# fanzhongyi/ExploreMultiModal

Measured on AMD Instinct MI355X. Metric: image-text pairs/sec fwd+bwd, VLMo-Base, 1/2/4/8 MI355X; % bf16 MFMA roofline, higher is better.
Workload: dtype bf16

## Files before the change

### exploremultimodal_amd/csrc/attention.hip

```cpp
#include "common.h"
#include "vlmo_hip.h"

namespace {

struct AttnArgs {
    const bf16* qkv;
    const bf16* ctx;
    const bf16* dctx;
    bf16* out;
    float* lse;
    float* qvsum;
    const int32_t* seg;
    const int32_t* keymask;
    int lse_stride, heads, d;
    float scale, scale_log2e;
    uint32_t drop_thresh, drop_cmp;
    float inv_keep;
    uint64_t seed;
    int bh0;
};

#define LOG2E 1.4426950408889634f
#define LN2 0.6931471805599453f

__device__ __forceinline__ int att_off(int row, int ch) {
    return 1024 * (row >> 3) + 512 * (ch >> 2) + 64 * (row & 7) + 16 * ((ch & 3) ^ ((row >> 2) & 3));
}

template <int NWAVES>
__device__ __forceinline__ void stage_image(const bf16* base, int ld, int col0, const int* rowidx, char* img, int ninstr,
                                            int wave, int lane) {
    const int chhi = lane >> 5, rowlo = (lane >> 2) & 7, pc = lane & 3;
    for (int ii = wave; ii < ninstr; ii += NWAVES) {
        const int row = ii * 8 + rowlo;
        const int ch = chhi * 4 + (pc ^ ((row >> 2) & 3));
        glds16(base + (size_t)rowidx[row] * ld + col0 + ch * 8, img + ii * 1024);
    }
}

#define ATT_G 0x9E3779B1u
#define ATT_G512 ((uint32_t)(512ull * ATT_G))
__device__ __forceinline__ uint32_t att_key(uint64_t seed, int bh) {
    return hash32((uint32_t)seed ^ ((uint32_t)bh * 0x9E3779B9u)) + (uint32_t)(seed >> 32);
}
__device__ __forceinline__ uint32_t att_mix(uint32_t x) {
    x ^= x >> 15;
    x *= 0x7feb352du;
    return x;
}

__device__ __forceinline__ bf16x8 row_frag(const char* img, int row_base, int ks, int lane) {
    return *(const bf16x8*)(img + att_off(row_base + (lane & 31), 2 * ks + (lane >> 5)));
}
__device__ __forceinline__ bf16x8 tr_frag(const char* img, int rb, int cb, int lane) {
    const int g = lane >> 4, q = (lane >> 2) & 3, pp = lane & 3, h = lane >> 5;
    const int col = cb + 16 * (g & 1) + 4 * pp;
    const int r0 = rb + 4 * h + q;
    const bf16x4 lo = lds_tr4<bf16>(img + att_off(r0, col >> 3) + (col & 7) * 2);
    const bf16x4 hi = lds_tr4<bf16>(img + att_off(r0 + 8, col >> 3) + (col & 7) * 2);
    return bf16x8{lo[0], lo[1], lo[2], lo[3], hi[0], hi[1], hi[2], hi[3]};
}

__device__ __forceinline__ f32x16 zero16() {
    f32x16 z;
#pragma unroll
    for (int i = 0; i < 16; ++i) z[i] = 0.f;
    return z;
}

struct SeqRows {
    int rowA, lenA, rowB, N;
    __device__ __forceinline__ SeqRows(const int32_t* seg, int sidx)
        : rowA(seg[4 * sidx + 0]), lenA(seg[4 * sidx + 1]), rowB(seg[4 * sidx + 2]), N(seg[4 * sidx + 1] + seg[4 * sidx + 3]) {}
    __device__ __forceinline__ SeqRows(const int32_t* seg, int sidx, int cap)
        : rowA(seg[4 * sidx + 0]), lenA(min(max(seg[4 * sidx + 1], 0), cap)), rowB(seg[4 * sidx + 2]),
          N(lenA + min(max(seg[4 * sidx + 3], 0), cap - lenA)) {
        if (N == 0) rowA = 1;
    }
    __device__ __forceinline__ int row(int tok) const {
        tok = min(tok, N - 1);
        return tok < lenA ? rowA + tok : rowB + (tok - lenA);
    }
};

__device__ __forceinline__ float key_bias(const int32_t* keymask, int row, int i, int N) {
    return (i < N && (!keymask || keymask[row] != 0)) ? 0.f : -INFINITY;
}

__device__ __forceinline__ void setup_rows(const SeqRows& sr, const int32_t* keymask, int npad, int* rowidx, float* kbias) {
    for (int i = threadIdx.x; i < npad; i += blockDim.x) {
        const int row = sr.row(i);
// ... 377 lines not shown

__device__ __forceinline__ float half_wave_total(float v) {
    float s_ = v + dpp_mov<0x111, 0xf, 0xf>(v);
    s_ += dpp_mov<0x112, 0xf, 0xf>(v);
    s_ += dpp_mov<0x113, 0xf, 0xf>(v);
    s_ += dpp_mov<0x114, 0xf, 0xe>(s_);
    s_ += dpp_mov<0x118, 0xf, 0xc>(s_);
    s_ += dpp_mov<0x142, 0xa, 0xf>(s_);
    return s_;
}
__device__ __forceinline__ void colsum_tile(const f32x16& t, float w, float scale, float* acc, int lane) {
    const int h = lane >> 5;
#pragma unroll
    for (int r = 0; r < 16; ++r) {
        const float v = half_wave_total(t[r] * w);
        if ((lane & 31) == 31) atomicAdd(acc + (r & 3) + 8 * (r >> 2) + 4 * h, v * scale);
    }
}
__device__ __forceinline__ void colsum_tiles(const f32x16* t, float w, float scale, float* acc, int lane) {
#pragma unroll
    for (int dt = 0; dt < 2; ++dt) colsum_tile(t[dt], w, scale, acc + dt * 32, lane);
}

__device__ __forceinline__ int slot_off(int k, int q) {
    return k * 64 + ((((q >> 2) ^ (k >> 1)) & 7) << 3) + (q & 3) * 2;
}
template <bool FRINGE>
__global__ __launch_bounds__(512) void attn_bwd1_kernel(const AttnArgs a, const int NPAD) {
    const int IMG = NPAD * 128;
    extern __shared__ __attribute__((aligned(16))) char smem[];
    char* Qimg = smem;
    char* Dimg = smem + IMG;
    char* Kimg = smem + 2 * IMG;
    const int nt = NPAD >> 5;
    char* slots = smem + 3 * IMG;
    float* kbias = (float*)(slots + 2 * nt * 2048);
    float* nlq = kbias + NPAD;
    float* ndl = nlq + NPAD;
    float* csum = ndl + NPAD;
    char* V8img = (char*)(csum + 128);

    const int lane = threadIdx.x & 63;
    const int w = __builtin_amdgcn_readfirstlane(threadIdx.x >> 6);
    const int nw = blockDim.x >> 6;
    const int bh = blockIdx.x, sidx = bh / a.heads, hd = bh % a.heads;
    const int ld = 3 * a.d;
    const SeqRows sr(a.seg, sidx);
    const int N = sr.N;
    const int nq = (N + 31) >> 5;
    const int nc = FRINGE ? min(nq, 8) : nq;
    for (int ii = w; ii < nq * 4; ii += nw) {
        const int chhi = lane >> 5, rowlo = (lane >> 2) & 7, pc = lane & 3;
        const int row = ii * 8 + rowlo;
        const int ch = chhi * 4 + (pc ^ ((row >> 2) & 3));
        const size_t r = (size_t)sr.row(row);
        glds16(a.qkv + r * ld + hd * 64 + ch * 8, Qimg + ii * 1024);
        glds16(a.qkv + r * ld + a.d + hd * 64 + ch * 8, Kimg + ii * 1024);
        glds16(a.dctx + r * a.d + hd * 64 + ch * 8, Dimg + ii * 1024);
    }
    if (FRINGE && nq > 8 && w >= 4) {
        const int chhi = lane >> 5, rowlo = (lane >> 2) & 7, pc = lane & 3;
        const int row = 256 + (w - 4) * 8 + rowlo;
        const int ch = chhi * 4 + (pc ^ ((row >> 2) & 3));
        glds16(a.qkv + (size_t)sr.row(row) * ld + 2 * a.d + hd * 64 + ch * 8, V8img + (w - 4) * 1024);
    }
    const int l31 = lane & 31, h = lane >> 5;
    const bool active = w < nc;
    const int ki = w * 32 + l31;
    const int krow = sr.row(ki);
    bf16x8 vf[4];
    if (active) {
        const bf16* kp = a.qkv + (size_t)krow * ld + a.d + hd * 64 + 8 * h;
#pragma unroll
        for (int s = 0; s < 4; ++s) vf[s] = *(const bf16x8*)(kp + a.d + 16 * s);
    }
    for (int i = threadIdx.x; i < 128; i += blockDim.x) csum[i] = 0.f;
    const float keep_prob = 1.f / a.inv_keep;
    const float inv_scale = 1.f / a.scale;
    for (int i = threadIdx.x; i < NPAD; i += blockDim.x) {
        float dl = 0.f, lq = INFINITY;
        const int row = sr.row(i);
        const float kb = key_bias(a.keymask, row, i, N);
        if (i < N) {
            const size_t o = (size_t)row * a.d + hd * 64;
            bf16x8 x[8], y[8];
#pragma unroll
            for (int c = 0; c < 8; ++c) {
                x[c] = *(const bf16x8*)(a.ctx + o + 8 * c);
                y[c] = *(const bf16x8*)(a.dctx + o + 8 * c);
            }
            lq = a.lse[(size_t)bh * a.lse_stride + i];
#pragma unroll
            for (int c = 0; c < 8; ++c)
#pragma unroll
                for (int j = 0; j < 8; ++j) dl += (float)x[c][j] * (float)y[c][j];
        }
        kbias[i] = kb;
        ndl[i] = -dl * keep_prob;
        nlq[i] = -lq * inv_scale;
    }
    asm volatile("s_waitcnt vmcnt(0)" ::: "memory");
    __syncthreads();

    const uint32_t akey = att_key(a.seed, bh + a.bh0);
    const float out_scale = a.scale * a.inv_keep;
    const float c_l2 = a.scale_log2e;
    const float kb_own = kbias[min(ki, NPAD - 1)];
    const uint32_t rl_own = (uint32_t)ki * ATT_G + akey + (uint32_t)(4 * h) * ATT_G512;
    f32x16 dK[2] = {zero16(), zero16()}, dV[2] = {zero16(), zero16()}, dQ[2] = {zero16(), zero16()};

    const int xq = (l31 >> 2) & 3;
    const int rf0 = 1024 * (l31 >> 3) + 64 * (l31 & 7) + 16 * (h ^ xq);
    const int rf1 = 1024 * (l31 >> 3) + 64 * (l31 & 7) + 16 * ((2 + h) ^ xq);
    const int tg = (lane >> 4) & 1, tq = (lane >> 2) & 3, tp = lane & 3;
    const int trl = 64 * (4 * h + tq) + 16 * ((2 * tg + (tp >> 1)) ^ h) + 8 * (tp & 1);
    const int trh = 1024 + 64 * (4 * h + tq) + 16 * ((2 * tg + (tp >> 1)) ^ ((2 + h) & 3)) + 8 * (tp & 1);
    auto rfrag = [&](const char* img_rb, int s) __attribute__((always_inline)) -> bf16x8 {
        return *(const bf16x8*)(img_rb + 512 * (s >> 1) + ((s & 1) ? rf1 : rf0));
    };
    auto tfrag = [&](const char* img_rb, int dt) __attribute__((always_inline)) -> bf16x8 {
        const bf16x4 lo = lds_tr4<bf16>(img_rb + 512 * dt + trl);
        const bf16x4 hi = lds_tr4<bf16>(img_rb + 512 * dt + trh);
        return bf16x8{lo[0], lo[1], lo[2], lo[3], hi[0], hi[1], hi[2], hi[3]};
    };
    const int sw0 = slot_off(l31, 4 * h), sw1 = slot_off(l31, 8 + 4 * h);
    const int srl = slot_off(4 * h + tq, 16 * tg + 4 * tp), srh = slot_off(8 + 4 * h + tq, 16 * tg + 4 * tp);
    auto sfrag = [&](const char* slot, int s2) __attribute__((always_inline)) -> bf16x8 {
        const bf16x4 lo = lds_tr4<bf16>(slot + 1024 * s2 + srl);
        const bf16x4 hi = lds_tr4<bf16>(slot + 1024 * s2 + srh);
        return bf16x8{lo[0], lo[1], lo[2], lo[3], hi[0], hi[1], hi[2], hi[3]};
    };

    bf16x8 qa[4], da[4], pf[2], sf[2];
    f32x16 S, dP;
    auto fetch_a = [&](int qt_) __attribute__((always_inline)) {
#pragma unroll
        for (int s = 0; s < 4; ++s) {
            qa[s] = rfrag(Qimg + qt_ * 4096, s);
            da[s] = rfrag(Dimg + qt_ * 4096, s);
        }
    };
    auto qtile = [&](int t_) __attribute__((always_inline)) {
        int q_ = w + t_;
        return q_ >= nc ? q_ - nc : q_;
    };
    auto stage_sdp = [&](int qt, const char* ktile, const bf16x8 (&vfr)[4]) __attribute__((always_inline)) {
        dP = zero16();
#pragma unroll
        for (int g4 = 0; g4 < 4; ++g4) {
            const f32x4 l4 = *(const f32x4*)(nlq + qt * 32 + 8 * g4 + 4 * h);
#pragma unroll
            for (int e = 0; e < 4; ++e) S[4 * g4 + e] = l4[e];
        }
#pragma unroll
        for (int s = 0; s < 4; ++s) {
            S = Elem<bf16>::mfma(qa[s], rfrag(ktile, s), S);
            dP = Elem<bf16>::mfma(da[s], vfr[s], dP);
        }
        __builtin_amdgcn_sched_barrier(0);
    };
    auto stage_valu_dvdk = [&](int qt, char* myslot, float kb, uint32_t rl, f32x16 (&dV)[2],
                               f32x16 (&dK)[2]) __attribute__((always_inline)) {
        bf16x8 dtr[2], qtr[2];
#pragma unroll
        for (int dt = 0; dt < 2; ++dt) {
            dtr[dt] = tfrag(Dimg + qt * 4096, dt);
            qtr[dt] = tfrag(Qimg + qt * 4096, dt);
        }
        __builtin_amdgcn_sched_barrier(0);
        if (a.drop_thresh) {
            const uint32_t rqt = rl + (uint32_t)(qt * 32) * ATT_G512;
#pragma unroll
            for (int g4 = 0; g4 < 4; ++g4) {
                const f32x4 nd = *(const f32x4*)(ndl + qt * 32 + 8 * g4 + 4 * h);
#pragma unroll
                for (int e = 0; e < 4; ++e) {
                    const int i = 4 * g4 + e;
                    const float p = __builtin_amdgcn_exp2f(fmaf(S[i], c_l2, kb));
// ... 175 lines not shown
        }
        __syncthreads();
        if (w < 4) add(w);
        if (w >= 1 && w < 4) put(w);
        __syncthreads();
        if (w == 0) {
            add(1), add(2), add(3);
            if (k8 < N) {
                store_tile(dK, out_scale, row8, a.d);
                store_tile(dV, a.inv_keep, row8, 2 * a.d);
            }
            if (a.qvsum) colsum_tiles(dV, wt8, a.inv_keep, csum + 64, lane);
        }
    } else if (active && ki < N) {
        bf16* op = a.out + (size_t)krow * ld + hd * 64 + 4 * h;
#pragma unroll
        for (int dt = 0; dt < 2; ++dt)
#pragma unroll
            for (int g4 = 0; g4 < 4; ++g4) {
                bf16x4 oq = {(bf16)(dQ[dt][4 * g4 + 0] * out_scale), (bf16)(dQ[dt][4 * g4 + 1] * out_scale),
                             (bf16)(dQ[dt][4 * g4 + 2] * out_scale), (bf16)(dQ[dt][4 * g4 + 3] * out_scale)};
                bf16x4 ok = {(bf16)(dK[dt][4 * g4 + 0] * out_scale), (bf16)(dK[dt][4 * g4 + 1] * out_scale),
                             (bf16)(dK[dt][4 * g4 + 2] * out_scale), (bf16)(dK[dt][4 * g4 + 3] * out_scale)};
                bf16x4 ov = {(bf16)(dV[dt][4 * g4 + 0] * a.inv_keep), (bf16)(dV[dt][4 * g4 + 1] * a.inv_keep),
                             (bf16)(dV[dt][4 * g4 + 2] * a.inv_keep), (bf16)(dV[dt][4 * g4 + 3] * a.inv_keep)};
                *(bf16x4*)(op + dt * 32 + 8 * g4) = oq;
                *(bf16x4*)(op + a.d + dt * 32 + 8 * g4) = ok;
                *(bf16x4*)(op + 2 * a.d + dt * 32 + 8 * g4) = ov;
            }
    }
    if (a.qvsum) {
        if (active && !(FRINGE && nq > 8)) {
            const float wt = ki < N ? 1.f : 0.f;
            colsum_tiles(dQ, wt, out_scale, csum, lane);
            colsum_tiles(dV, wt, a.inv_keep, csum + 64, lane);
        }
        __syncthreads();
        for (int i = threadIdx.x; i < 128; i += blockDim.x) {
            float* dst = a.qvsum + (size_t)sidx * 2 * a.d + (i >> 6) * a.d + hd * 64 + (i & 63);
            *dst = csum[i];
        }
    }
}

#define ATT_LW 8
#define ATT_LCH 4
#define ATT_LBUF (ATT_LCH * 4096)
#define ATT_LMAX 1024
#define ATT_LDS_FWD (4 * ATT_LBUF + ATT_LMAX * 4)
#define ATT_LDS_BWD (4 * ATT_LBUF + 3 * ATT_LMAX * 4 + ATT_LW * 64 * 4)

__device__ __forceinline__ uint32_t att_stride(int N) { return N > 512 ? 1024u : 512u; }

__device__ __forceinline__ void stage_chunk(const bf16* pa, int lda, const bf16* pb, int ldb, const SeqRows& sr, int t0,
                                            int nt, char* ia, char* ib, int w, int lane) {
    const int chhi = lane >> 5, rowlo = (lane >> 2) & 7, pc = lane & 3;
    for (int ii = w; ii < nt * 4; ii += ATT_LW) {
        const int row = t0 * 32 + ii * 8 + rowlo;
        const int ch = chhi * 4 + (pc ^ ((row >> 2) & 3));
        const size_t r = (size_t)sr.row(row);
        glds16(pa + r * lda + ch * 8, ia + ii * 1024);
        glds16(pb + r * ldb + ch * 8, ib + ii * 1024);
    }
}

__device__ __forceinline__ void colsum_wave(const f32x16* t, float wt, float* part, int lane) {
    const int h = lane >> 5;
#pragma unroll
    for (int dt = 0; dt < 2; ++dt)
#pragma unroll
        for (int r = 0; r < 16; ++r) {
            const float v = half_wave_total(t[dt][r] * wt);
            if ((lane & 31) == 31) part[dt * 32 + (r & 3) + 8 * (r >> 2) + 4 * h] += v;
        }
}

__device__ __forceinline__ void bwd_row_constants(const AttnArgs& a, const SeqRows& sr, int bh, int hd, int npad,
                                                  float* lseq, float* delta, float* kbias) {
    const float keep_prob = 1.f / a.inv_keep;
    for (int i = threadIdx.x; i < npad; i += blockDim.x) {
        float dl = 0.f, lq = INFINITY;
        const int row = sr.row(i);
        if (i < sr.N) {
            const size_t o = (size_t)row * a.d + hd * 64;
            bf16x8 x[8], y[8];
#pragma unroll
            for (int c = 0; c < 8; ++c) {
                x[c] = *(const bf16x8*)(a.ctx + o + 8 * c);
                y[c] = *(const bf16x8*)(a.dctx + o + 8 * c);
            }
            lq = a.lse[(size_t)bh * a.lse_stride + i] * LOG2E;
#pragma unroll
            for (int c = 0; c < 8; ++c)
#pragma unroll
                for (int j = 0; j < 8; ++j) dl += (float)x[c][j] * (float)y[c][j];
        }
        delta[i] = dl * keep_prob;
        lseq[i] = lq;
        if (kbias) kbias[i] = key_bias(a.keymask, row, i, sr.N);
    }
}

__global__ __launch_bounds__(512) void attn_fwd_long_kernel(const AttnArgs a) {
    extern __shared__ __attribute__((aligned(16))) char smem[];
    char* ring = smem;
    float* kbias = (float*)(smem + 4 * ATT_LBUF);

    const int lane = threadIdx.x & 63;
    const int w = __builtin_amdgcn_readfirstlane(threadIdx.x >> 6);
    const int bh = blockIdx.x, sidx = bh / a.heads, hd = bh % a.heads;
    const int ld = 3 * a.d;
    const SeqRows sr(a.seg, sidx);
    const int N = sr.N;
    if (N <= 0) return;
    const int nq = (N + 31) >> 5, nch = (nq + ATT_LCH - 1) / ATT_LCH, nrounds = (nq + ATT_LW - 1) / ATT_LW;
    const bf16* kb0 = a.qkv + a.d + hd * 64;
    const bf16* vb0 = a.qkv + 2 * a.d + hd * 64;
    stage_chunk(kb0, ld, vb0, ld, sr, 0, min(ATT_LCH, nq), ring, ring + ATT_LBUF, w, lane);
    for (int i = threadIdx.x; i < nq * 32; i += blockDim.x) kbias[i] = key_bias(a.keymask, sr.row(i), i, N);

    const int l31 = lane & 31, h = lane >> 5;
    const uint32_t akey = att_key(a.seed, bh + a.bh0);
    const uint32_t stride = att_stride(N);
    int qi = 0, qrow = 0;
    uint32_t rq = 0;
    bf16x8 qf[4];
    float m_run = -INFINITY, l_run = 0.f;
    f32x16 O[2] = {zero16(), zero16()};
    const int nsteps = nrounds * nch;
    for (int j = 0; j < nsteps; ++j) {
        const int rd = j / nch, c = j - rd * nch;
        asm volatile("s_waitcnt vmcnt(0)" ::: "memory");
        __syncthreads();
        if (j + 1 < nsteps) {
            const int t0 = ((j + 1) % nch) * ATT_LCH;
            char* nb = ring + ((j + 1) & 1) * 2 * ATT_LBUF;
            stage_chunk(kb0, ld, vb0, ld, sr, t0, min(ATT_LCH, nq - t0), nb, nb + ATT_LBUF, w, lane);
        }
        const char* Kc = ring + (j & 1) * 2 * ATT_LBUF;
        const char* Vc = Kc + ATT_LBUF;
        const int qt = rd * ATT_LW + w;
        if (qt >= nq) continue;
        if (c == 0) {
            qi = qt * 32 + l31;
            qrow = sr.row(qi);
            rq = ((uint32_t)qi * stride + 4u * h) * ATT_G + akey;
            const bf16* qp = a.qkv + (size_t)qrow * ld + hd * 64 + 8 * h;
#pragma unroll
            for (int s = 0; s < 4; ++s) qf[s] = *(const bf16x8*)(qp + 16 * s);
            m_run = -INFINITY, l_run = 0.f;
            O[0] = zero16(), O[1] = zero16();
        }
        const int c0 = c * ATT_LCH;
        f32x16 S[ATT_LCH];
        float mx = -INFINITY;
#pragma unroll
        for (int cc = 0; cc < ATT_LCH; ++cc) {
            S[cc] = zero16();
            const int kt = c0 + cc;
            if (kt < nq) {
#pragma unroll
                for (int s = 0; s < 4; ++s) S[cc] = Elem<bf16>::mfma(row_frag(Kc, cc * 32, s, lane), qf[s], S[cc]);
#pragma unroll
                for (int g4 = 0; g4 < 4; ++g4) {
                    const f32x4 kb = *(const f32x4*)(kbias + kt * 32 + 8 * g4 + 4 * h);
#pragma unroll
                    for (int e = 0; e < 4; ++e) {
                        const float t = S[cc][4 * g4 + e] * a.scale_log2e + kb[e];
                        S[cc][4 * g4 + e] = t;
                        mx = fmaxf(mx, t);
                    }
                }
            }
        }
        mx = fmaxf(mx, __shfl_xor(mx, 32, 64));
        const float m_new = fmaxf(m_run, mx);
        const bool dead = (m_new == -INFINITY);
        const float alpha = dead ? 1.f : __builtin_amdgcn_exp2f(m_run - m_new);
// ... 486 lines not shown
}

int check_common(const char* fn, const void* qkv, const int32_t* seg, int num_seq, int heads, int d, int max_len,
                 int cap) {
    VLMO_CHECK_ARG(qkv && seg, "%s: null pointer", fn);
    VLMO_CHECK_ARG(num_seq > 0 && heads > 0, "%s: empty problem", fn);
    VLMO_CHECK_ARG(d == heads * 64, "%s: head_dim must be 64 (d=%d, heads=%d)", fn, d, heads);
    VLMO_CHECK_ARG(max_len > 0 && max_len <= cap, "%s: sequence length %d exceeds this build's limit %d", fn, max_len, cap);
    return 0;
}

AttnArgs make_args(const void* qkv, const int32_t* seg, const int32_t* keymask, const float* lse, int lse_stride, int heads,
                   int d, float scale, uint32_t drop_thresh, float inv_keep, uint64_t seed, int mask_seq0) {
    AttnArgs a{};
    a.qkv = (const bf16*)qkv;
    a.lse = (float*)lse;
    a.seg = seg;
    a.keymask = keymask;
    a.lse_stride = lse_stride;
    a.heads = heads;
    a.d = d;
    a.scale = scale;
    a.scale_log2e = scale * LOG2E;
    a.drop_thresh = drop_thresh;
    a.drop_cmp = drop_thresh >= 65536u ? 0xFFFFFFFFu : drop_thresh << 16;
    a.inv_keep = drop_thresh ? inv_keep : 1.f;
    a.seed = seed;
    a.bh0 = mask_seq0 * heads;
    return a;
}

int run_map(const char* fn, const void* qkv, const void* dctx, const int32_t* seg, int num_seq, const int32_t* keymask,
            float* out, int heads, int d, int seq_len, int q0, int nq, int kind, int head_mean, float scale,
            hipStream_t stream) {
    if (int rc = check_common(fn, qkv, seg, num_seq, heads, d, seq_len, ATT_LMAX)) return rc;
    VLMO_CHECK_ARG(q0 >= 0 && nq >= 1 && q0 <= seq_len - nq, "%s: query rows [%d, %d + %d) outside [0, %d)", fn, q0, q0, nq,
                   seq_len);
    MapArgs a{};
    a.qkv = (const bf16*)qkv;
    a.dctx = (const bf16*)dctx;
    a.seg = seg;
    a.keymask = keymask;
    a.out = out;
    a.heads = heads;
    a.d = d;
    a.seq_len = seq_len;
    a.q0 = q0;
    a.nq = nq;
    a.kind = kind;
    a.head_mean = head_mean != 0;
    a.scale_log2e = scale * LOG2E;
    const int gx = num_seq * (a.head_mean ? 1 : heads);
    const int rounds = ((nq + 31) / 32 + ATT_PW - 1) / ATT_PW;
    const int gy = std::min(rounds, std::max(1, (768 + gx - 1) / gx));
    a.tiles_per_block = ATT_PW * ((rounds + gy - 1) / gy);
    launch_map(a, gx, (rounds * ATT_PW + a.tiles_per_block - 1) / a.tiles_per_block, stream);
    VLMO_CHECK_LAUNCH(fn);
    return 0;
}

}

extern "C" int vlmo_attn_fwd(const void* qkv, const int32_t* seg, int num_seq, const int32_t* keymask, void* ctx,
                             float* lse, int lse_stride, int heads, int d, int max_len, float scale,
                             uint32_t drop_thresh, float inv_keep, uint64_t seed, int mask_seq0, hipStream_t stream) {
    if (int rc = check_common("vlmo_attn_fwd", qkv, seg, num_seq, heads, d, max_len, 1024)) return rc;
    VLMO_CHECK_ARG(ctx, "vlmo_attn_fwd: null ctx");
    VLMO_CHECK_ARG(!lse || lse_stride >= max_len, "vlmo_attn_fwd: lse_stride too small");
    AttnArgs a = make_args(qkv, seg, keymask, lse, lse_stride, heads, d, scale, drop_thresh, inv_keep, seed, mask_seq0);
    a.out = (bf16*)ctx;
    const int nt = (max_len + 31) / 32, nb = num_seq * heads;
    if (max_len > 512) {
        launch_fwd_long(a, nb, stream);
        VLMO_CHECK_LAUNCH("vlmo_attn_fwd(long)");
        return 0;
    }
    if (nt == 9) launch_fwd1_fringe(a, max_len, nb, stream);
    else if (nt < 9) launch_fwd1(a, nt, nb, stream);
    else launch_fwd(a, nt, nb, stream);
    VLMO_CHECK_LAUNCH("vlmo_attn_fwd");
    return 0;
}

extern "C" int vlmo_attn_bwd(const void* qkv, const void* ctx, const void* dctx, const float* lse, int lse_stride,
                             const int32_t* seg, int num_seq, const int32_t* keymask, void* dqkv, float* qv_colsum,
                             int heads, int d, int max_len, float scale, uint32_t drop_thresh, float inv_keep,
                             uint64_t seed, int mask_seq0, hipStream_t stream) {
    if (int rc = check_common("vlmo_attn_bwd", qkv, seg, num_seq, heads, d, max_len, 1024)) return rc;
    VLMO_CHECK_ARG(ctx && dctx && lse && dqkv, "vlmo_attn_bwd: null pointer");
    VLMO_CHECK_ARG(lse_stride >= max_len, "vlmo_attn_bwd: lse_stride too small");
    AttnArgs a = make_args(qkv, seg, keymask, lse, lse_stride, heads, d, scale, drop_thresh, inv_keep, seed, mask_seq0);
    a.ctx = (const bf16*)ctx;
    a.dctx = (const bf16*)dctx;
    a.out = (bf16*)dqkv;
    a.qvsum = qv_colsum;
    const int nt = (max_len + 31) / 32, nb = num_seq * heads;
    if (max_len > 288) {
        launch_bwd_long(a, nb, stream);
        VLMO_CHECK_LAUNCH("vlmo_attn_bwd(long)");
        return 0;
    }
    const int rc = nt > 8 ? launch_bwd1<true>(a, nt, nb, stream) : launch_bwd1<false>(a, nt, nb, stream);
    VLMO_CHECK_ARG(rc == 0, "vlmo_attn_bwd: %d tokens do not fit the LDS of one CU", max_len);
    VLMO_CHECK_LAUNCH("vlmo_attn_bwd");
    return 0;
}

extern "C" int vlmo_attn_probs(const void* qkv, const int32_t* seg, int num_seq, const int32_t* keymask, float* probs,
                               int heads, int d, int seq_len, int q0, int nq, int head_mean, float scale,
                               hipStream_t stream) {
    VLMO_CHECK_ARG(probs, "vlmo_attn_probs: null probs");
    return run_map("vlmo_attn_probs", qkv, nullptr, seg, num_seq, keymask, probs, heads, d, seq_len, q0, nq, 0, head_mean,
                   scale, stream);
}

extern "C" int vlmo_attn_gradcam(const void* qkv, const void* dctx, const int32_t* seg, int num_seq, const int32_t* keymask,
                                 float* out, int heads, int d, int seq_len, int q0, int nq, int kind, int head_mean,
                                 float scale, hipStream_t stream) {
    VLMO_CHECK_ARG(dctx && out, "vlmo_attn_gradcam: null dctx or out");
    VLMO_CHECK_ARG(kind == VLMO_GRADCAM_CAM || kind == VLMO_GRADCAM_ATTN_GRAD || kind == VLMO_GRADCAM_GRAD,
                   "vlmo_attn_gradcam: unknown kind %d", kind);
    return run_map("vlmo_attn_gradcam", qkv, dctx, seg, num_seq, keymask, out, heads, d, seq_len, q0, nq, kind, head_mean,
                   scale, stream);
}
```

### exploremultimodal_amd/csrc/block.hip

```cpp
#include "common.h"
#include "vlmo_hip.h"
#include <algorithm>
#include <map>
#include <vector>

namespace {
constexpr int GELU_DERIV = 4;


struct Events {
    std::vector<hipEvent_t> pool;
    hipEvent_t get(size_t i) {
        while (pool.size() <= i) {
            hipEvent_t e = nullptr;
            (void)hipEventCreateWithFlags(&e, hipEventDisableTiming);
            pool.push_back(e);
        }
        return pool[i];
    }
};
Events& events() {
    static thread_local std::map<int, Events> per_device;
    int dev = 0;
    (void)hipGetDevice(&dev);
// ... 69 lines not shown
        w2[x] = b->w2[x];
        VlmoEpilogue& f = e2[x] = epi();
        f.out = bp(b->x2, r0, d, 4);
        f.ldo = d;
        f.out2 = b->need_bwd ? bp(b->zd2, r0, d, 2) : nullptr;
        f.ld2 = d;
        f.bias = b->b2[x];
        f.gamma = b->g2;
        f.resid = (const float*)bp((const void*)b->x1, r0, d, 4);
        f.row_scale = b->row_index ? b->rs2 : (b->rs2 ? b->rs2 + r0 : nullptr);
        f.row_index = b->row_index ? b->row_index + r0 : nullptr;
        f.drop_thresh = b->drop_thresh;
        f.inv_keep = b->inv_keep;
        f.seed = b->seed + 21 + 2 * x;
    }
    TRY(vlmo_gemm_nt_grouped(VLMO_EPI_BIAS_GELU, VLMO_BF16, b->tile, b->n_experts, a1, d, w1, d, rows, hid, d, e1, st));
    TRY(vlmo_gemm_nt_grouped(VLMO_EPI_RESID, VLMO_BF16, b->tile, b->n_experts, a2, hid, w2, hid, rows, d, hid, e2, st));
    return 0;
}

}

extern "C" int vlmo_side_stream_create(int low_priority, const uint32_t* cu_mask, int cu_mask_words, hipStream_t* out) {
    VLMO_CHECK_ARG(out, "vlmo_side_stream_create: null out");
    hipError_t rc;
    if (cu_mask && cu_mask_words > 0) {
        rc = hipExtStreamCreateWithCUMask(out, (uint32_t)cu_mask_words, cu_mask);
    } else {
        int least = 0, greatest = 0;
        (void)hipDeviceGetStreamPriorityRange(&least, &greatest);
        rc = hipStreamCreateWithPriority(out, hipStreamNonBlocking, low_priority ? least : 0);
    }
    if (rc != hipSuccess) {
        vlmo_set_error("vlmo_side_stream_create: %s", hipGetErrorString(rc));
        return (int)rc;
    }
    return 0;
}

namespace {

struct Deferred {
    std::vector<VlmoTnProblem> tn;
    std::vector<VlmoColJob> col;
    std::vector<int> blocks;
    bool store = false;
};

void push_col(Deferred& D, const VlmoColJob& j) {
    if (j.src && j.rows > 0) D.col.push_back(j);
}
void push_tn(Deferred& D, const void* A, int lda, const void* B, int ldb, float* C, int ldc, int M, int N1, int N2) {
    D.tn.push_back(VlmoTnProblem{A, B, C, lda, ldb, ldc, M, N1, N2, 1.f, D.store ? 0 : 1});
}

struct StackWs {
    int64_t ln2;
    int64_t resid[2];
    int64_t ln1;
    int64_t colpart;
    int64_t qv;
    int64_t total;
    int64_t slot;
};
StackWs stack_ws_layout(int M, int d, int hidden, int max_seqs) {
    StackWs w{};
    w.slot = reduce_ws_need(2 * d) / 4;
    w.ln2 = 0;
    w.resid[0] = w.ln2 + 2 * w.slot;
    w.resid[1] = w.resid[0] + w.slot;
    w.ln1 = w.resid[1] + w.slot;
    w.colpart = w.ln1 + 2 * w.slot;
    w.qv = w.colpart + (int64_t)((M + 15) / 16 + 1) * hidden;
    w.total = w.qv + (int64_t)max_seqs * 2 * d;
    return w;
}
int block_seqs(const VlmoBlockDesc* b) {
    int n = 0;
    for (int a = 0; a < b->n_attn; ++a) n += b->nseq[a];
    return n;
}

int check_block_bwd(const VlmoBlockDesc* b, int i) {
    VLMO_CHECK_ARG(b->dx2 && b->dx1 && b->dx0, "vlmo_stack_bwd: block %d: null gradient buffers", i);
    VLMO_CHECK_ARG(b->n_experts >= 1 && b->n_experts <= 2 && b->n_attn >= 1 && b->n_attn <= 2,
                   "vlmo_stack_bwd: block %d: 1..2 experts and attention launches per block", i);
    VLMO_CHECK_ARG(b->M > 0 && b->exp_rows[0] >= 0 && (b->n_experts == 1 || b->exp_rows[1] >= 0) &&
                       (int64_t)b->exp_rows[0] + (b->n_experts == 2 ? b->exp_rows[1] : 0) <= b->M,
                   "vlmo_stack_bwd: block %d: expert rows exceed M = %d", i, b->M);
    const int64_t need = stack_ws_layout(b->M, b->d, b->hidden, block_seqs(b)).total * 4;
    VLMO_CHECK_ARG(b->ws_main && b->ws_bytes >= need,
                   "vlmo_stack_bwd: block %d: column workspace of %lld bytes is too small: need %lld bytes = "
                   "vlmo_stack_bwd_ws_bytes(%d, %d, %d, %d)",
                   i, (long long)b->ws_bytes, (long long)need, b->M, b->d, b->hidden, block_seqs(b));
    return 0;
}

int block_dgrad_chain(const VlmoBlockDesc* b, hipStream_t st, Deferred& D, const VlmoBlockDesc* below, bool skip_resid,
                      bool* fused_below) {
    const int M = b->M, d = b->d, hid = b->hidden;
    const int nseq_all = block_seqs(b);
    const StackWs W = stack_ws_layout(M, d, hid, nseq_all);
    const int64_t slot_bytes = W.slot * 4;
    float* const ws = b->ws_main;
    const void *ag[4], *wg[4], *af[4], *wf[4];
    int32_t rows[4];
    VlmoEpilogue eg[4], ef[4];
    float* colpart = ws + W.colpart;
    for (int x = 0; x < b->n_experts; ++x) {
        const size_t r0 = b->exp_row0[x];
        const int n = rows[x] = b->exp_rows[x];
        if (!skip_resid) {
            VlmoColJob fold{};
            TRY(resid_bwd_launch(b->dx2 + r0 * d, bp(b->zd2, r0, d, 2), b->g2,
                                 b->row_index ? b->rs2 : (b->rs2 ? b->rs2 + r0 : nullptr),
                                 b->row_index ? b->row_index + r0 : nullptr, bp(b->dz2, r0, d, 2), b->dg2, b->db2[x], n, d,
                                 b->drop_thresh, b->inv_keep, b->seed + 21 + 2 * x, ws + W.resid[x], slot_bytes, &fold, st));
            push_col(D, fold);
        }
        ag[x] = bp(b->dz2, r0, d, 2);
        wg[x] = b->w2T[x];
        VlmoEpilogue& e = eg[x] = epi();
        e.out = bp(b->du, r0, hid, 2);
        e.ldo = hid;
        e.aux = bp(b->u, r0, hid, 2);
        e.ld2 = hid;
        e.drop_thresh = b->drop_thresh;
        e.inv_keep = b->inv_keep;
        e.seed = b->seed + 20 + 2 * x;
        e.relu = GELU_DERIV;
        if (b->db1[x]) {
            const int nblk16 = (n + 15) / 16;
            e.colpart = colpart;
            push_col(D, fold_job(colpart, hid, nblk16, hid, hid, b->db1[x]));
            colpart += (int64_t)nblk16 * hid;
        }
        af[x] = bp(b->du, r0, hid, 2);
        wf[x] = b->w1T[x];
        VlmoEpilogue& f = ef[x] = epi();
        f.out = bp(b->dy2, r0, d, 2);
        f.ldo = d;
        push_tn(D, bp(b->dz2, r0, d, 2), d, bp(b->h, r0, hid, 2), hid, b->dw2[x], hid, n, d, hid);
        push_tn(D, bp(b->du, r0, hid, 2), hid, bp(b->y2, r0, d, 2), d, b->dw1[x], d, n, hid, d);
    }
    TRY(vlmo_gemm_nt_grouped(VLMO_EPI_DGELU, VLMO_BF16, b->tile, b->n_experts, ag, d, wg, d, rows, hid, d, eg, st));
    TRY(vlmo_gemm_nt_grouped(VLMO_EPI_BIAS, VLMO_BF16, b->tile, b->n_experts, af, hid, wf, hid, rows, d, hid, ef, st));
    {
        VlmoColJob fold{};
        TRY(ln_bwd_fold(b->dy2, b->x1, b->n2w, b->mean2, b->rstd2, b->dx2, b->dx1, b->dn2w, b->dn2b, b->zd1, b->g1, b->rs1,
                        b->row_index, b->dz1, b->dg1, b->dproj_b, b->drop_thresh, b->inv_keep, b->seed + 1, M, d, ws + W.ln2,
                        2 * slot_bytes, &fold, st));
        push_col(D, fold);
    }
    {
        VlmoEpilogue e = epi();
        e.out = b->dctx;
        e.ldo = d;
        TRY(vlmo_gemm_nt(VLMO_EPI_BIAS, VLMO_BF16, b->tile, b->dz1, d, b->proj_wT, d, M, d, d, &e, st));
    }
    const float scale = 1.0f / sqrtf((float)(d / b->heads));
    float* const qvsum = ws + W.qv;
    for (int a = 0, s0 = 0; a < b->n_attn; s0 += b->nseq[a], ++a)
        TRY(vlmo_attn_bwd(b->qkv, b->ctx, b->dctx, b->lse[a], b->lse_stride[a], b->seg[a], b->nseq[a], b->keymask,
                          b->dqkv, qvsum + (size_t)s0 * 2 * d, b->heads, d, b->maxlen[a], scale, b->attn_drop_thresh,
                          b->attn_inv_keep, b->seed + 11 + b->attn_seed_idx[a], b->attn_seq0[a], st));
    push_tn(D, b->dz1, d, b->ctx, d, b->dproj_w, d, M, d, d);
    push_tn(D, b->dqkv, 3 * d, b->y1, d, b->dqkv_w, d, M, 3 * d, d);
    push_col(D, fold_job(qvsum, 2 * d, nseq_all, 2 * d, d, b->dqkv_b, b->dqkv_b + 2 * d));
    {
        VlmoEpilogue e = epi();
        e.out = b->dy1;
        e.ldo = d;
        TRY(vlmo_gemm_nt(VLMO_EPI_BIAS, VLMO_BF16, b->tile, b->dqkv, 3 * d, b->qkv_wT, 3 * d, M, d, 3 * d, &e, st));
    }
    const VlmoBlockDesc* n = below;
    *fused_below = n && n->M == M && n->d == d && n->dx2 == b->dx0 && n->zd2 && n->dz2 && n->exp_row0[0] == 0 &&
                   (n->n_experts == 1 ? n->exp_rows[0] == M
                                      : (n->exp_row0[1] == n->exp_rows[0] && n->exp_rows[0] + n->exp_rows[1] == M));
    VlmoColJob fold{};
    if (*fused_below) {
        const int seg = n->n_experts == 1 ? M : n->exp_row0[1];
        float* wsf = ws + W.ln1;
        int nb0 = 0;
        TRY(ln_resid_seg_bwd(b->dy1, b->x, b->n1w, b->mean1, b->rstd1, b->dx1, b->dx0, b->dn1w, b->dn1b, n->zd2, n->g2,
                             n->rs2, n->row_index, n->dz2, n->dg2, n->drop_thresh, n->inv_keep, n->seed + 21, n->seed + 23,
                             seg, M, d, wsf, 2 * slot_bytes, &fold, &nb0, st));
        push_col(D, fold);
        if (n->db2[0]) push_col(D, fold_job(wsf + 3 * d, 4 * d, nb0, d, d, n->db2[0]));
        if (n->n_experts == 2 && n->db2[1])
            push_col(D, fold_job(wsf + 3 * d + (size_t)nb0 * 4 * d, 4 * d, fold.rows - nb0, d, d, n->db2[1]));
    } else {
        TRY(ln_bwd_fold(b->dy1, b->x, b->n1w, b->mean1, b->rstd1, b->dx1, b->dx0, b->dn1w, b->dn1b, nullptr, nullptr, nullptr,
                        nullptr, nullptr, nullptr, nullptr, 0, 1.f, 0, M, d, ws + W.ln1, slot_bytes, &fold, st));
        push_col(D, fold);
    }
    return 0;
}

}

extern "C" int64_t vlmo_stack_bwd_ws_bytes(int M, int d, int hidden, int max_seqs) {
    return stack_ws_layout(M, d, hidden, max_seqs).total * 4;
}

extern "C" int vlmo_stack_fwd(const VlmoStackDesc* s, hipStream_t st) {
    VLMO_CHECK_ARG(s && s->blocks && s->n_blocks >= 1, "vlmo_stack_fwd: empty stack");
    for (int i = 0; i < s->n_blocks; ++i)
        if (int rc = block_fwd(&s->blocks[i], st)) return rc;
    return 0;
}

extern "C" int vlmo_stack_bwd(const VlmoStackDesc* s, hipStream_t st) {
    VLMO_CHECK_ARG(s && s->blocks && s->n_blocks >= 1, "vlmo_stack_bwd: empty stack");
    const int nb = s->n_blocks;
    for (int i = 0; i < nb; ++i) TRY(check_block_bwd(&s->blocks[i], i));
    const int batch = s->wgrad_batch >= 1 ? s->wgrad_batch : 1;
    const int nsets = s->n_tmp_sets >= 1 ? s->n_tmp_sets : 1;
    hipStream_t side = s->side_stream ? s->side_stream : st;
    const bool two = side != st;
    VLMO_CHECK_ARG(!two || nsets > batch || nb <= nsets,
                   "vlmo_stack_bwd: %d temporary sets cannot cover deferred batches of %d blocks", nsets, batch);
    Events& ev = events();
    Deferred D;
    D.store = s->wgrad_store != 0;
    std::vector<int> batch_of(nb, -1);
    int n_batches = 0, waited_upto = -1;
    auto flush = [&]() -> int {
        if (D.blocks.empty()) return 0;
        if (two) {
            hipEvent_t f = ev.get(2 * n_batches);
            (void)hipEventRecord(f, st);
            (void)hipStreamWaitEvent(side, f, 0);
        }
        std::stable_sort(D.tn.begin(), D.tn.end(), [](const VlmoTnProblem& a, const VlmoTnProblem& b) { return a.M > b.M; });
        TRY(vlmo_gemm_tn_multi(VLMO_BF16, D.tn.data(), (int)D.tn.size(), side));
        TRY(vlmo_colwork_multi(VLMO_BF16, D.col.data(), (int)D.col.size(), side));
        if (two) (void)hipEventRecord(ev.get(2 * n_batches + 1), side);
        if (s->grad_ready)
            for (int i : D.blocks)
                if (s->grad_ready[i]) (void)hipEventRecord((hipEvent_t)s->grad_ready[i], side);
        ++n_batches;
        D.tn.clear();
        D.col.clear();
        D.blocks.clear();
        return 0;
    };
    auto set_free = [&](int kk) -> int {
        if (!two || kk < nsets || kk >= nb) return 0;
// ... 44 lines not shown
```

### exploremultimodal_amd/csrc/common.h

```cpp
#pragma once
#include <hip/hip_runtime.h>
#include <stdint.h>
#include <type_traits>
#include "vlmo_hip.h"

typedef __bf16 bf16;
typedef _Float16 f16;
typedef __attribute__((ext_vector_type(8))) __bf16 bf16x8;
typedef __attribute__((ext_vector_type(4))) __bf16 bf16x4;
typedef __attribute__((ext_vector_type(2))) __bf16 bf16x2;
typedef __attribute__((ext_vector_type(8))) _Float16 f16x8;
typedef __attribute__((ext_vector_type(4))) _Float16 f16x4;
typedef __attribute__((ext_vector_type(16))) float f32x16;
typedef __attribute__((ext_vector_type(4))) float f32x4;
typedef __attribute__((ext_vector_type(2))) float f32x2;

#define LDS_PTR(p) ((__attribute__((address_space(3))) void*)(p))
#define GLB_PTR(p) ((const __attribute__((address_space(1))) void*)(p))

void vlmo_set_error(const char* fmt, ...);
#define VLMO_CHECK_ARG(cond, ...)                         \
    do {                                                  \
        if (!(cond)) {                                    \
            vlmo_set_error(__VA_ARGS__);                  \
// ... 84 lines not shown
#endif
    __device__ __forceinline__ void init(const void* base) {
#if defined(__HIP_DEVICE_COMPILE__)
        r = __builtin_amdgcn_make_buffer_rsrc((void*)base, 0, 0x7FFFFFFF, 0x00020000);
#endif
    }
    __device__ __forceinline__ void load16(void* lds_wave_base, uint32_t lane_off, int scalar_off) const {
#if defined(__HIP_DEVICE_COMPILE__)
        __builtin_amdgcn_raw_ptr_buffer_load_lds(r, LDS_PTR(lds_wave_base), 16, lane_off, scalar_off, 0, 0);
#endif
    }
};

template <typename T>
__device__ __forceinline__ typename Elem<T>::v4 lds_tr4(const void* p);
template <>
__device__ __forceinline__ bf16x4 lds_tr4<bf16>(const void* p) {
    return __builtin_amdgcn_ds_read_tr16_b64_v4bf16(
        (__attribute__((address_space(3))) bf16x4*)(p));
}
template <>
__device__ __forceinline__ f16x4 lds_tr4<f16>(const void* p) {
    typedef __attribute__((__vector_size__(4 * sizeof(__fp16)))) __fp16 hv4;
    const hv4 r = __builtin_amdgcn_ds_read_tr16_b64_v4f16((__attribute__((address_space(3))) hv4*)(p));
    return __builtin_bit_cast(f16x4, r);
}

__device__ __forceinline__ uint32_t hash32(uint32_t x) {
    x ^= x >> 16;
    x *= 0x7feb352du;
    x ^= x >> 15;
    x *= 0x846ca68bu;
    x ^= x >> 16;
    return x;
}
__device__ __forceinline__ uint32_t drop_half(uint64_t seed, uint64_t group_idx, int half) {
    const uint32_t i = (uint32_t)(group_idx * 2 + half);
    return hash32((i ^ (uint32_t)seed) * 0x9E3779B9u + (uint32_t)(seed >> 32));
}
__device__ __forceinline__ uint64_t drop_bits4(uint64_t seed, uint64_t group_idx) {
    return (uint64_t)drop_half(seed, group_idx, 0) | ((uint64_t)drop_half(seed, group_idx, 1) << 32);
}
__device__ __forceinline__ bool drop_keep(uint64_t bits, int j, uint32_t thresh) {
    return ((uint32_t)(bits >> (16 * j)) & 0xFFFFu) >= thresh;
}
__device__ __forceinline__ bool drop_keep1(uint64_t seed, uint64_t group_idx, int j, uint32_t thresh) {
    return ((drop_half(seed, group_idx, j >> 1) >> (16 * (j & 1))) & 0xFFFFu) >= thresh;
}

__device__ __forceinline__ float norm_cdf_from(float x, float e) {
    const float t = __builtin_amdgcn_rcpf(fmaf(0.3275911f * 0.70710678118654752f, fabsf(x), 1.0f));
    float poly = fmaf(0.5f * 1.061405429f, t, 0.5f * -1.453152027f);
    poly = fmaf(poly, t, 0.5f * 1.421413741f);
    poly = fmaf(poly, t, 0.5f * -0.284496736f);
    poly = fmaf(poly, t, 0.5f * 0.254829592f);
    const float tail = poly * t * e;
    return x >= 0.f ? 1.0f - tail : tail;
}
__device__ __forceinline__ float gauss_from(float x) {
    return __builtin_amdgcn_exp2f(x * x * -0.72134752044448170f);
}
__device__ __forceinline__ float gelu_erf(float x) {
    const float e = gauss_from(x);
    return x * norm_cdf_from(x, e);
}
__device__ __forceinline__ float gelu_erf_grad(float x) {
    const float e = gauss_from(x);
    return norm_cdf_from(x, e) + x * 0.39894228040143268f * e;
}

template <int CTRL, int ROW_MASK, int BANK_MASK> __device__ __forceinline__ float dpp_mov(float v) {
    return __builtin_bit_cast(float, __builtin_amdgcn_update_dpp(0, __builtin_bit_cast(int, v), CTRL, ROW_MASK, BANK_MASK, false));
}
__device__ __forceinline__ float wave_sum(float v) {
    float s = v + dpp_mov<0x111, 0xf, 0xf>(v);
    s += dpp_mov<0x112, 0xf, 0xf>(v);
    s += dpp_mov<0x113, 0xf, 0xf>(v);
    s += dpp_mov<0x114, 0xf, 0xe>(s);
    s += dpp_mov<0x118, 0xf, 0xc>(s);
    s += dpp_mov<0x142, 0xa, 0xf>(s);
    s += dpp_mov<0x143, 0xc, 0xf>(s);
    return __builtin_bit_cast(float, __builtin_amdgcn_readlane(__builtin_bit_cast(int, s), 63));
}
__device__ __forceinline__ float wave_max(float v) {
#pragma unroll
    for (int o = 32; o > 0; o >>= 1) v = fmaxf(v, __shfl_xor(v, o, 64));
    return v;
}
```

### exploremultimodal_amd/csrc/gemm_common.h

```cpp
#pragma once
#include "common.h"
#include "vlmo_hip.h"

namespace {

struct GemmNT {
    const void* A;
    const void* B;
    int M, N, K, lda, ldb;
    VlmoEpilogue e;
    int cH, cW, cCin, ckw;
    const void* zero;
    int group_m;
    const void* A2;
    int lda2, k1;
    float seg_scale;
};

constexpr int MAX_GROUPS = 4;
struct GemmNTGroups {
    int ngroups;
    int t0[MAX_GROUPS + 1];
    GemmNT g[MAX_GROUPS];
};

struct RowAddr {
    size_t base;
    uint32_t off;
    template <typename U> __device__ __forceinline__ U* at(const void* p) const {
        return (U*)((char*)((U*)p + base) + off * (uint32_t)sizeof(U));
    }
};
template <typename T, bool NT = true> __device__ __forceinline__ void store4(T* p, float a, float b, float c, float d) {
    typedef typename Elem<T>::v4 v4;
    const v4 v = {(T)a, (T)b, (T)c, (T)d};
    if constexpr (NT)
        __builtin_nontemporal_store(v, (v4*)p);
    else
        *(v4*)p = v;
}
#define NT_LD(p) __builtin_nontemporal_load(p)
template <typename T> __device__ __forceinline__ f32x4 load4(const T* p);
template <> __device__ __forceinline__ f32x4 load4<bf16>(const bf16* p) {
    bf16x4 v = NT_LD((const bf16x4*)p);
    return f32x4{(float)v[0], (float)v[1], (float)v[2], (float)v[3]};
}
template <> __device__ __forceinline__ f32x4 load4<f16>(const f16* p) {
    f16x4 v = NT_LD((const f16x4*)p);
    return f32x4{(float)v[0], (float)v[1], (float)v[2], (float)v[3]};
}

__device__ __forceinline__ void pin4(f32x4& v) {
    asm volatile("" : "+v"(v[0]), "+v"(v[1]), "+v"(v[2]), "+v"(v[3]));
}

template <typename T, int EPI, int GD = -1>
__device__ __forceinline__ f32x4 epilogue4(const GemmNT& p, int gmb, int row, int gn, f32x4 v, f32x4 bias4,
                                           f32x4 gamma4, f32x4 ext, float rs, bool ok) {
    const VlmoEpilogue& e = p.e;
    v += bias4;
    const int gm = gmb + row;
    const RowAddr o{(size_t)gmb * e.ldo, (uint32_t)(row * e.ldo + gn)};
    const RowAddr o2{(size_t)gmb * e.ld2, (uint32_t)(row * e.ld2 + gn)};
    if constexpr (EPI == VLMO_EPI_BIAS) {
        const float lo = (e.relu & 1) ? 0.f : -INFINITY;
#pragma unroll
        for (int j = 0; j < 4; ++j) v[j] = fmaxf(v[j], lo);
        pin4(v);
        if (ok) store4<T>(o.at<T>(e.out), v[0], v[1], v[2], v[3]);
    } else if constexpr (EPI == VLMO_EPI_F32) {
        if (e.beta != 0.f) v += e.beta * ext;
        pin4(v);
        if (ok) *(f32x4*)o.at<float>(e.out) = v;
    } else if constexpr (EPI == VLMO_EPI_BIAS_GELU) {
        f32x4 h;
        if (GD >= 0 ? GD != 0 : (e.relu & 4) != 0) {
#pragma unroll
            for (int j = 0; j < 4; ++j) {
                const float u = v[j], ee = gauss_from(u), cdf = norm_cdf_from(u, ee);
                h[j] = u * cdf;
                v[j] = fmaf(u * 0.39894228040143268f, ee, cdf);
            }
            if (e.drop_thresh) {
                const uint64_t bits = drop_bits4(e.seed, ((uint64_t)gm * p.N + gn) >> 2);
#pragma unroll
                for (int j = 0; j < 4; ++j) {
                    const float m = drop_keep(bits, j, e.drop_thresh) ? e.inv_keep : 0.f;
                    h[j] *= m;
                    v[j] *= m;
                }
            }
        } else {
#pragma unroll
            for (int j = 0; j < 4; ++j) h[j] = gelu_erf(v[j]);
            if (e.drop_thresh) {
                const uint64_t bits = drop_bits4(e.seed, ((uint64_t)gm * p.N + gn) >> 2);
#pragma unroll
                for (int j = 0; j < 4; ++j) h[j] = drop_keep(bits, j, e.drop_thresh) ? h[j] * e.inv_keep : 0.f;
            }
        }
        pin4(v);
        pin4(h);
        if (ok) {
            store4<T>(o.at<T>(e.out), v[0], v[1], v[2], v[3]);
            store4<T>(o2.at<T>(e.out2), h[0], h[1], h[2], h[3]);
        }
    } else if constexpr (EPI == VLMO_EPI_RESID) {
        if (e.drop_thresh) {
            const uint64_t bits = drop_bits4(e.seed, ((uint64_t)gm * p.N + gn) >> 2);
#pragma unroll
            for (int j = 0; j < 4; ++j) v[j] = drop_keep(bits, j, e.drop_thresh) ? v[j] * e.inv_keep : 0.f;
        }
        f32x4 x2 = ext + gamma4 * v * rs;
        pin4(v);
        pin4(x2);
        if (ok) {
            if (e.out2) store4<T>(o2.at<T>(e.out2), v[0], v[1], v[2], v[3]);
            *(f32x4*)o.at<float>(e.out) = x2;
        }
    } else if constexpr (EPI == VLMO_EPI_DUAL) {
        v = v * e.beta + ext;
        pin4(v);
        if (ok) {
            store4<T>(o.at<T>(e.out), v[0], v[1], v[2], v[3]);
            if (e.out2)
                store4<T>((T*)e.out2 + (size_t)gm * e.ld2 + gn, fmaxf(v[0], 0.f), fmaxf(v[1], 0.f), fmaxf(v[2], 0.f),
                          fmaxf(v[3], 0.f));
        }
    } else if constexpr (EPI == VLMO_EPI_CE_BWD) {
        const int gmc = min(gm, p.M - 1);
        const float lse = e.resid[gmc], sc = e.row_scale[gmc];
        const int lab = e.row_index[gmc];
#pragma unroll
        for (int j = 0; j < 4; ++j)
            v[j] = (__builtin_amdgcn_exp2f((v[j] - lse) * 1.4426950408889634f) - (gn + j == lab ? 1.f : 0.f)) * sc;
        pin4(v);
        if (ok) store4<T>(o.at<T>(e.out), v[0], v[1], v[2], v[3]);
    } else if constexpr (EPI == VLMO_EPI_DGELU) {
        if (GD >= 0 ? GD != 0 : (e.relu & 4) != 0) {
            v *= ext;
        } else {
#pragma unroll
            for (int j = 0; j < 4; ++j) v[j] *= gelu_erf_grad(ext[j]);
            if (e.drop_thresh) {
                const uint64_t bits = drop_bits4(e.seed, ((uint64_t)gm * p.N + gn) >> 2);
#pragma unroll
                for (int j = 0; j < 4; ++j) v[j] = drop_keep(bits, j, e.drop_thresh) ? v[j] * e.inv_keep : 0.f;
            }
        }
        pin4(v);
        if (ok) store4<T>(o.at<T>(e.out), v[0], v[1], v[2], v[3]);
    }
    return v;
}

template <typename T, int EPI>
__device__ __forceinline__ f32x4 epilogue_ext(const GemmNT& p, int gmb, int rowc, int gnc) {
    const VlmoEpilogue& e = p.e;
    const f32x4 z = {0.f, 0.f, 0.f, 0.f};
    const RowAddr o{(size_t)gmb * e.ldo, (uint32_t)(rowc * e.ldo + gnc)};
    const RowAddr o2{(size_t)gmb * e.ld2, (uint32_t)(rowc * e.ld2 + gnc)};
    if constexpr (EPI == VLMO_EPI_RESID) {
        return NT_LD((const f32x4*)o.at<float>(e.resid));
    } else if constexpr (EPI == VLMO_EPI_DGELU) {
        return load4<T>(o2.at<T>(e.aux));
    } else if constexpr (EPI == VLMO_EPI_DUAL) {
        return e.resid ? load4<T>(o.at<T>(e.resid)) : z;
    } else if constexpr (EPI == VLMO_EPI_F32) {
        return e.beta != 0.f ? *(const f32x4*)o.at<float>(e.out) : z;
    } else {
        return z;
    }
}

__device__ __forceinline__ const void* uniform_ptr(const void* p) {
    const uint64_t v = (uint64_t)p;
    const uint32_t lo = __builtin_amdgcn_readfirstlane((uint32_t)v), hi = __builtin_amdgcn_readfirstlane((uint32_t)(v >> 32));
    return (const void*)(const __attribute__((address_space(1))) void*)(((uint64_t)hi << 32) | lo);
}

__device__ __forceinline__ int uniform_i(int v) { return __builtin_amdgcn_readfirstlane(v); }
__device__ __forceinline__ float uniform_f(float v) {
    return __builtin_bit_cast(float, __builtin_amdgcn_readfirstlane(__builtin_bit_cast(int, v)));
}

__device__ __forceinline__ int xcd_remap(int bid, int nwg) {
    const int q = nwg >> 3, r = nwg & 7, x = bid & 7;
    const int base = (x < r) ? x * (q + 1) : r * (q + 1) + (x - r) * q;
    return base + (bid >> 3);
}

template <int BK> __device__ __forceinline__ int nt_swz(int row) {
    return BK == 64 ? ((row >> 1) & 7) : ((row >> 2) & 3);
}

template <typename T, int BM, int BN, int WM, int WN, int EPI, bool CONV, int BK, int NSTG, bool PP = false>
__global__ __launch_bounds__(WM * WN * 64, 2) void gemm_nt_kernel(const GemmNTGroups gp) {
    typedef typename Elem<T>::v8 v8;
    constexpr bool SEG2 = __is_same(T, f16) && !CONV;
    constexpr int NW = WM * WN;
    constexpr int TM = BM / WM / 32, TN = BN / WN / 32;
    constexpr int ROWB = BK * 2, CPR = ROWB / 16, SRPI = 1024 / ROWB, KS = BK / 16;
    constexpr int A_BYTES = BM * ROWB, B_BYTES = BN * ROWB, STAGE = A_BYTES + B_BYTES;
    constexpr int NA = BM / SRPI / NW, NB = BN / SRPI / NW;
    static_assert(BM % (SRPI * NW) == 0 && BN % (SRPI * NW) == 0, "tile/wave mismatch");
    static_assert(NW * 32 * TN * 32 * 4 <= NSTG * STAGE, "epilogue LDS must fit in the ring");
    extern __shared__ __attribute__((aligned(16))) char smem[];

    const int tid = threadIdx.x, lane = tid & 63;
    const int wave = __builtin_amdgcn_readfirstlane(tid >> 6);
    const int wm = wave / WN, wn = wave % WN;
    const int lid_all = xcd_remap(blockIdx.x, gridDim.x);
    auto locate = [&](int la, int& gi_, int& m0_, int& n0_) {
        int g = 0;
#pragma unroll
        for (int q = 1; q < MAX_GROUPS; ++q)
            if (q < gp.ngroups && la >= gp.t0[q]) g = q;
        g = __builtin_amdgcn_readfirstlane(g);
        const GemmNT& r = gp.g[g];
        const int M_ = uniform_i(r.M), N_ = uniform_i(r.N);
        const int tiles_n = (N_ + BN - 1) / BN, tiles_m = (M_ + BM - 1) / BM;
        const int lid = la - uniform_i(gp.t0[g]);
        const int gmr = uniform_i(r.group_m);
        const int gm_ = gmr > 0 ? gmr : 1;
        const int per_group = gm_ * tiles_n;
        const int first_m = (lid / per_group) * gm_;
        const int gsz = min(tiles_m - first_m, gm_);
        const int in_g = lid % per_group;
        gi_ = g;
        m0_ = (first_m + in_g % gsz) * BM;
        n0_ = (in_g / gsz) * BN;
    };
    const T* a_src[NA];
    const T* b_src[NB];
    int a_yx[NA];
    auto point = [&](int gi_, int m0_, int n0_) {
        const GemmNT& r = gp.g[gi_];
        const T* A_ = (const T*)uniform_ptr(r.A);
        const T* B_ = (const T*)uniform_ptr(r.B);
        const int M_ = uniform_i(r.M), N_ = uniform_i(r.N), lda_ = uniform_i(r.lda), ldb_ = uniform_i(r.ldb);
#pragma unroll
        for (int i = 0; i < NA; ++i) {
            const int rr = (i * NW + wave) * SRPI + lane / CPR;
            const int c = (lane % CPR) ^ nt_swz<BK>(rr);
            const int gr = min(m0_ + rr, M_ - 1);
            a_src[i] = A_ + (size_t)gr * lda_ + c * 8;
            if constexpr (CONV) {
                const int cH = uniform_i(r.cH), cW = uniform_i(r.cW);
                const int pix = gr % (cH * cW);
                a_yx[i] = ((pix / cW) << 16) | (pix % cW);
            }
        }
#pragma unroll
        for (int i = 0; i < NB; ++i) {
            const int rr = (i * NW + wave) * SRPI + lane / CPR;
// ... 126 lines not shown
            }
        }
    }
    stage(0, 0);
#pragma unroll
    for (int i = 0; i < TM; ++i)
#pragma unroll
        for (int j = 0; j < TN; ++j)
#pragma unroll
            for (int k = 0; k < 16; ++k) acc[i][j][k] = 0.f;
    if constexpr (PP) {
        static_assert(NSTG == 2 && WM == 2 && KS == 4, "ping-pong schedule: 2 buffers, 2 row groups, BK = 64");
        v8 af[2][TM], bf[2][TN];
        auto read_half = [&](const char* s_, int hf) {
#pragma unroll
            for (int q = 0; q < 2; ++q) {
                const int coff = ((2 * (2 * hf + q) + h) ^ swz) << 4;
#pragma unroll
                for (int i = 0; i < TM; ++i) af[q][i] = *(const v8*)(s_ + a_row_off + i * 32 * ROWB + coff);
#pragma unroll
                for (int j = 0; j < TN; ++j) bf[q][j] = *(const v8*)(s_ + b_row_off + j * 32 * ROWB + coff);
            }
            if constexpr (CONV && sizeof(T) == 2 && __is_same(T, f16)) {
                if (pp->e.relu & 2) {
                    const v8 z = {0, 0, 0, 0, 0, 0, 0, 0};
#pragma unroll
                    for (int q = 0; q < 2; ++q)
#pragma unroll
                        for (int i = 0; i < TM; ++i) af[q][i] = __builtin_elementwise_max(af[q][i], z);
                }
            }
        };
        auto mfma_half = [&]() {
            __builtin_amdgcn_s_setprio(1);
#pragma unroll
            for (int q = 0; q < 2; ++q)
#pragma unroll
                for (int i = 0; i < TM; ++i)
#pragma unroll
                    for (int j = 0; j < TN; ++j) acc[i][j] = Elem<T>::mfma(af[q][i], bf[q][j], acc[i][j]);
            __builtin_amdgcn_s_setprio(0);
        };
        auto bar = [&]() {
            __builtin_amdgcn_sched_barrier(0);
            asm volatile("s_waitcnt lgkmcnt(0)" ::: "memory");
            __builtin_amdgcn_s_barrier();
            asm volatile("" ::: "memory");
            __builtin_amdgcn_sched_barrier(0);
        };
        asm volatile("s_waitcnt vmcnt(0)" ::: "memory");
        __builtin_amdgcn_s_barrier();
        if (wm == 1) bar();
        for (int kt = 0; kt < nk; ++kt) {
            const char* cur = smem + (kt & 1) * STAGE;
            const bool more = kt + 1 < nk;
            seg_boundary(kt);
            read_half(cur, 0);
            if (more) stage((kt + 1) & 1, kt + 1);
            bar();
            mfma_half();
            bar();
            read_half(cur, 1);
            if (more && wm == 1) asm volatile("s_waitcnt vmcnt(0)" ::: "memory");
            bar();
            mfma_half();
            if (more && wm == 0) asm volatile("s_waitcnt vmcnt(0)" ::: "memory");
            bar();
        }
        if (wm == 0) bar();
    } else {
        static_assert(NSTG == 2, "two LDS buffers");
        for (int kt = 0; kt < nk; ++kt) {
            asm volatile("s_waitcnt vmcnt(0)" ::: "memory");
            __syncthreads();
            if (kt + 1 < nk) stage((kt + 1) & 1, kt + 1);
            seg_boundary(kt);
            compute(smem + (kt & 1) * STAGE);
        }
    }

    __syncthreads();
    constexpr int ROWF = TN * 32;
    constexpr int LPR = TN * 8, RPI = 64 / LPR;
    float* ep = (float*)(smem + wave * (32 * ROWF * 4));
    const int rrow = lane / LPR, rcol = (lane % LPR) * 4;
    const int gn = n0 + wn * (BN / WN) + rcol;
    const bool col_ok = gn < p.N;
    const int gnc = col_ok ? gn : 0;
    f32x4 bias4 = {0.f, 0.f, 0.f, 0.f}, gamma4 = {1.f, 1.f, 1.f, 1.f};
    if (p.e.bias) bias4 = *(const f32x4*)(p.e.bias + gnc);
    if (EPI == VLMO_EPI_RESID && p.e.gamma) gamma4 = *(const f32x4*)(p.e.gamma + gnc);
    f32x4 csum = {0.f, 0.f, 0.f, 0.f};
#pragma unroll
    for (int i = 0; i < TM; ++i) {
        constexpr int NIT = 32 / RPI;
        const int gmb = __builtin_amdgcn_readfirstlane(m0 + wm * (BM / WM) + i * 32);
        const int gmbc = min(gmb, p.M - 1);
        f32x4 ext[NIT];
        float rs[NIT];
        int ridx[NIT];
#pragma unroll
        for (int it = 0; it < NIT; ++it) {
            const int gmc = gmbc + min(it * RPI + rrow, p.M - 1 - gmbc);
            ridx[it] = (EPI == VLMO_EPI_RESID && p.e.row_scale && p.e.row_index) ? p.e.row_index[gmc] : gmc;
        }
#pragma unroll
        for (int it = 0; it < NIT; ++it) {
            const int rowc = min(it * RPI + rrow, p.M - 1 - gmbc);
            if constexpr (PRE) {
                const typename Elem<T>::v4 q = pre[i][it];
                ext[it] = p.e.resid ? f32x4{(float)q[0], (float)q[1], (float)q[2], (float)q[3]} : f32x4{0.f, 0.f, 0.f, 0.f};
            } else {
                ext[it] = epilogue_ext<T, EPI>(p, gmbc, rowc, gnc);
            }
            rs[it] = (EPI == VLMO_EPI_RESID && p.e.row_scale) ? p.e.row_scale[ridx[it]] : 1.f;
        }
#pragma unroll
        for (int j = 0; j < TN; ++j)
#pragma unroll
            for (int r = 0; r < 16; ++r)
                ep[((r & 3) + 8 * (r >> 2) + 4 * h) * ROWF + j * 32 + l31] = acc[i][j][r];
        __builtin_amdgcn_fence(__ATOMIC_RELEASE, "wavefront");
        __builtin_amdgcn_wave_barrier();
        __builtin_amdgcn_fence(__ATOMIC_ACQUIRE, "wavefront");
        f32x4 v[NIT];
#pragma unroll
        for (int it = 0; it < NIT; ++it) v[it] = *(const f32x4*)(ep + (it * RPI + rrow) * ROWF + rcol);
#pragma unroll
        for (int it = 0; it < NIT; ++it) {
            const int row = it * RPI + rrow;
            const int gm = gmb + row;
            if constexpr (EPI == VLMO_EPI_ARGMAX) {
                f32x4 vv = v[it] + bias4;
                float best = -INFINITY;
                int bi = 0x7fffffff;
#pragma unroll
                for (int j = 0; j < 4; ++j)
                    if (gn + j < p.N && vv[j] > best) {
                        best = vv[j];
                        bi = gn + j;
                    }
#pragma unroll
                for (int o = 1; o < LPR; o <<= 1) {
                    const float ob = __shfl_xor(best, o, 64);
                    const int oi = __shfl_xor(bi, o, 64);
                    if (ob > best || (ob == best && oi < bi)) {
                        best = ob;
                        bi = oi;
                    }
                }
                if ((lane % LPR) == 0 && gm < p.M && col_ok) {
                    const int chunk = (n0 + wn * (BN / WN)) / ROWF;
                    float* pv = (float*)p.e.out + ((size_t)gm * p.e.ldo + chunk) * 2;
                    pv[0] = best;
                    ((int*)pv)[1] = bi;
                }
            } else if constexpr (EPI == VLMO_EPI_CE) {
                f32x4 vv = v[it] + bias4;
                const int lab = (gm < p.M) ? p.e.row_index[gm] : -1;
                float best = -INFINITY, labv = -INFINITY;
                int bi = 0x7fffffff;
#pragma unroll
                for (int j = 0; j < 4; ++j)
                    if (gn + j < p.N) {
                        if (vv[j] > best) {
                            best = vv[j];
                            bi = gn + j;
                        }
                        if (gn + j == lab) labv = vv[j];
                    }
#pragma unroll
                for (int o = 1; o < LPR; o <<= 1) {
                    const float ob = __shfl_xor(best, o, 64);
                    const int oi = __shfl_xor(bi, o, 64);
                    if (ob > best || (ob == best && oi < bi)) {
                        best = ob;
                        bi = oi;
                    }
                    labv = fmaxf(labv, __shfl_xor(labv, o, 64));
                }
                float se = 0.f;
#pragma unroll
                for (int j = 0; j < 4; ++j)
                    if (gn + j < p.N) se += __builtin_amdgcn_exp2f((vv[j] - best) * 1.4426950408889634f);
#pragma unroll
                for (int o = 1; o < LPR; o <<= 1) se += __shfl_xor(se, o, 64);
                if ((lane % LPR) == 0 && gm < p.M && col_ok) {
                    const int chunk = (n0 + wn * (BN / WN)) / ROWF;
                    float* pv = (float*)p.e.out + ((size_t)gm * p.e.ldo + chunk) * 4;
                    pv[0] = best;
                    pv[1] = se;
                    ((int*)pv)[2] = bi;
                    pv[3] = labv;
                }
            } else {
                const bool ok = gm < p.M && col_ok;
                const f32x4 w = epilogue4<T, EPI>(p, gmb, row, gn, v[it], bias4, gamma4, ext[it], rs[it], ok);
                if constexpr (EPI == VLMO_EPI_DGELU) {
#pragma unroll
                    for (int j = 0; j < 4; ++j) csum[j] += ok ? w[j] : 0.f;
                }
            }
        }
        __builtin_amdgcn_fence(__ATOMIC_RELEASE, "wavefront");
        __builtin_amdgcn_wave_barrier();
        __builtin_amdgcn_fence(__ATOMIC_ACQUIRE, "wavefront");
        if constexpr (EPI == VLMO_EPI_DGELU) {
            if (p.e.colpart) {
#pragma unroll
                for (int o = LPR; o < 64; o <<= 1)
#pragma unroll
                    for (int j = 0; j < 4; ++j) csum[j] += __shfl_xor(csum[j], o, 64);
                const int blk = gmb >> 4;
                if (lane < LPR && col_ok && gmb < p.M) {
                    *(f32x4*)(p.e.colpart + (size_t)blk * p.N + gn) = csum;
                    if (gmb + 16 < p.M) *(f32x4*)(p.e.colpart + (size_t)(blk + 1) * p.N + gn) = f32x4{0.f, 0.f, 0.f, 0.f};
                }
                csum = f32x4{0.f, 0.f, 0.f, 0.f};
            }
        }
    }
}

template <typename T, int BM, int BN, int WM, int WN, bool CONV = false, int BK = 64, int NSTG = 2, bool PP = false,
          unsigned EMASK = 0xFFFFFFFFu>
int launch_nt(int epi, GemmNTGroups& p, hipStream_t st) {
    int tiles = 0;
    for (int q = 0; q < p.ngroups; ++q) {
        p.t0[q] = tiles;
        tiles += ((p.g[q].M + BM - 1) / BM) * ((p.g[q].N + BN - 1) / BN);
    }
    for (int q = p.ngroups; q <= MAX_GROUPS; ++q) p.t0[q] = tiles;
    constexpr int LDS = NSTG * (BM + BN) * BK * 2;
    dim3 grid(tiles), block(WM * WN * 64);
#define VLMO_LAUNCH_EPI(E)                                                                     \
    case E:                                                                                    \
    if constexpr (((EMASK >> E) & 1u) == 0) {                                                  \
        known = false;                                                                         \
    } else {                                                                                   \
        auto k = gemm_nt_kernel<T, BM, BN, WM, WN, E, CONV, BK, NSTG, PP>;                                        \
        if (LDS > 65536) {                                                                     \
            static DeviceOnce attr_set;              \
            if (attr_set.first())                                                              \
                (void)hipFuncSetAttribute((const void*)k, hipFuncAttributeMaxDynamicSharedMemorySize, LDS); \
        }                                                                                      \
        hipLaunchKernelGGL(k, grid, block, LDS, st, p);                                        \
    } break;
    bool known = true;
    switch (epi) {
        VLMO_LAUNCH_EPI(VLMO_EPI_BIAS)
        VLMO_LAUNCH_EPI(VLMO_EPI_F32)
        VLMO_LAUNCH_EPI(VLMO_EPI_DUAL)
        default:
            if constexpr (!CONV) {
                switch (epi) {
                    VLMO_LAUNCH_EPI(VLMO_EPI_BIAS_GELU)
                    VLMO_LAUNCH_EPI(VLMO_EPI_RESID)
                    VLMO_LAUNCH_EPI(VLMO_EPI_DGELU)
                    VLMO_LAUNCH_EPI(VLMO_EPI_ARGMAX)
                    VLMO_LAUNCH_EPI(VLMO_EPI_CE)
                    VLMO_LAUNCH_EPI(VLMO_EPI_CE_BWD)
                    default:
                        known = false;
                }
            } else {
                known = false;
            }
    }
    if (!known) {
        vlmo_set_error("vlmo_gemm_nt/conv: unsupported epilogue %d", epi);
        return -1;
    }
#undef VLMO_LAUNCH_EPI
    VLMO_CHECK_LAUNCH("vlmo_gemm_nt");
    return 0;
}

}

namespace vlmo_prof {
struct ProfRec;
struct ProfScope {
    ProfRec* r = nullptr;
    hipStream_t st;
    ProfScope(int tag, double flops, hipStream_t s);
    ~ProfScope();
};
}
using vlmo_prof::ProfScope;

extern "C" __attribute__((visibility("hidden"))) int launch_nt16_height(int h16, int epi, GemmNTGroups& gp,
                                                                        hipStream_t stream);
```

### exploremultimodal_amd/csrc/gemm_nt.hip

```cpp
#include "gemm_common.h"
#include <mutex>
#include <vector>

namespace vlmo_prof {
struct ProfRec {
    hipEvent_t a, b;
    int tag;
    double flops;
};
struct Prof {
    std::vector<ProfRec> recs;
    size_t used = 0;
    bool on = false;
    std::mutex mu;
} g_prof;

ProfScope::ProfScope(int tag, double flops, hipStream_t s) : st(s) {
    if (!g_prof.on) return;
    std::lock_guard<std::mutex> lk(g_prof.mu);
    if (g_prof.used < g_prof.recs.size()) {
        r = &g_prof.recs[g_prof.used++];
        r->tag = tag;
        r->flops = flops;
        (void)hipEventRecord(r->a, st);
    }
}
ProfScope::~ProfScope() {
    if (r) (void)hipEventRecord(r->b, st);
}

extern "C" int vlmo_profile_start(int max_records) {
    std::lock_guard<std::mutex> lk(g_prof.mu);
    while ((int)g_prof.recs.size() < max_records) {
        ProfRec r{};
        if (hipEventCreate(&r.a) != hipSuccess || hipEventCreate(&r.b) != hipSuccess) {
            vlmo_set_error("vlmo_profile_start: hipEventCreate failed");
            return -1;
        }
        g_prof.recs.push_back(r);
    }
    g_prof.used = 0;
    g_prof.on = true;
    return 0;
}

extern "C" int vlmo_profile_stop(int ntags, double* ms, double* flops, int64_t* launches) {
    std::lock_guard<std::mutex> lk(g_prof.mu);
    g_prof.on = false;
    for (int i = 0; i < ntags; ++i) {
        ms[i] = 0;
        flops[i] = 0;
        launches[i] = 0;
    }
    for (size_t i = 0; i < g_prof.used; ++i) {
        const ProfRec& r = g_prof.recs[i];
        float t = 0.f;
        if (r.tag < 0 || r.tag >= ntags || hipEventElapsedTime(&t, r.a, r.b) != hipSuccess) continue;
        ms[r.tag] += t;
        flops[r.tag] += r.flops;
        launches[r.tag] += 1;
    }
    return (int)g_prof.used;
}
}

namespace {
int check_nt(int epi, const void* A, int lda, const void* B, int ldb, int M, int N, int K, const VlmoEpilogue* e) {
    VLMO_CHECK_ARG(A && B && e, "vlmo_gemm_nt: null operand");
    VLMO_CHECK_ARG(M > 0 && N > 0 && K > 0, "vlmo_gemm_nt: empty problem M=%d N=%d K=%d", M, N, K);
    VLMO_CHECK_ARG(K % 64 == 0, "vlmo_gemm_nt: K=%d must be a multiple of 64", K);
    VLMO_CHECK_ARG(N % 4 == 0, "vlmo_gemm_nt: N=%d must be a multiple of 4", N);
    VLMO_CHECK_ARG(lda % 8 == 0 && ldb % 8 == 0 && lda >= K && ldb >= K, "vlmo_gemm_nt: bad lda/ldb %d/%d", lda, ldb);
    VLMO_CHECK_ARG(e->out && (epi == VLMO_EPI_ARGMAX || epi == VLMO_EPI_CE || (e->ldo >= N && e->ldo % 4 == 0)), "vlmo_gemm_nt: bad output / ldo");
    VLMO_CHECK_ARG(epi != VLMO_EPI_CE || (e->ldo >= (N + 63) / 64 && e->row_index), "vlmo_gemm_nt: cross-entropy epilogue needs labels and ldo >= chunks");
    VLMO_CHECK_ARG(epi != VLMO_EPI_CE_BWD || (e->resid && e->row_scale && e->row_index), "vlmo_gemm_nt: cross-entropy backward needs lse, row scale, labels");
    VLMO_CHECK_ARG(epi != VLMO_EPI_BIAS_GELU || (e->out2 && e->ld2 >= N), "vlmo_gemm_nt: gelu epilogue needs out2");
    VLMO_CHECK_ARG(epi != VLMO_EPI_ARGMAX || e->ldo >= (N + 63) / 64, "vlmo_gemm_nt: argmax partial buffer too narrow");
    VLMO_CHECK_ARG(epi != VLMO_EPI_RESID || e->resid, "vlmo_gemm_nt: residual epilogue needs resid");
    VLMO_CHECK_ARG(epi != VLMO_EPI_DGELU || (e->aux && e->ld2 >= N), "vlmo_gemm_nt: dgelu epilogue needs aux");
    return 0;
}

int run_nt(int epi, int dtype, int tile, GemmNTGroups& gp, hipStream_t stream) {
    VLMO_CHECK_ARG(dtype == VLMO_BF16 || dtype == VLMO_F16, "vlmo_gemm_nt: dtype must be bf16 or f16");
    const int tile_in = tile;
    long Mtot = 0;
    for (int q = 0; q < gp.ngroups; ++q) Mtot += gp.g[q].M;
    const int N = gp.g[0].N, K = gp.g[0].K;
    if (tile < 0) {
        tile = (K >= 1536 && Mtot >= 2048 && N >= 512) ? 3 : 0;
        if (tile == 0 && K >= 512 && N >= 512 && Mtot >= 2048) {
            long t256 = 0;
            for (int q = 0; q < gp.ngroups; ++q) t256 += (long)((gp.g[q].M + 255) / 256) * ((N + 255) / 256);
            if (t256 <= 256) tile = 3;
        }
        long t256_all = 0;
        for (int q = 0; q < gp.ngroups; ++q) t256_all += (long)((gp.g[q].M + 255) / 256) * ((N + 255) / 256);
        const bool few_tiles = t256_all <= 128;
        if (few_tiles) tile = 0;
        if (tile == 0 && dtype == VLMO_BF16 && (epi == VLMO_EPI_BIAS || epi == VLMO_EPI_BIAS_GELU) && K <= 1024 && N >= 2048 && Mtot >= 4096)
            tile = 4;
        if (!few_tiles && dtype == VLMO_BF16 && (epi == VLMO_EPI_BIAS || epi == VLMO_EPI_BIAS_GELU || epi == VLMO_EPI_RESID || epi == VLMO_EPI_DGELU) && K >= 1024) {
            long t256 = 0, t192n = 0;
            for (int q = 0; q < gp.ngroups; ++q) {
                t256 += (long)((gp.g[q].M + 255) / 256) * ((N + 255) / 256);
                t192n += (long)((gp.g[q].M + 191) / 192) * ((N + 255) / 256);
            }
            const long e256 = ((t256 + 255) / 256) * 256, e192 = ((t192n + 255) / 256) * 192;
            if (e192 * 10 <= e256 * 9) tile = 8;
        }
    }
    if ((tile == 0 || tile == 3 || tile == 4 || tile == 8) && dtype == VLMO_BF16 && !gp.g[0].k1 && !gp.g[0].ckw &&
        (epi == VLMO_EPI_BIAS || epi == VLMO_EPI_BIAS_GELU || epi == VLMO_EPI_RESID || epi == VLMO_EPI_DGELU) && N >= 512 && K >= 512 &&
        Mtot * (long)N >= 40 * 65536l && tile_in < 0) {
        auto count = [&](int bm, int bn) {
            long t = 0;
            for (int q = 0; q < gp.ngroups; ++q) t += (long)((gp.g[q].M + bm - 1) / bm) * ((N + bn - 1) / bn);
            return t;
        };
        double cur;
        if (tile == 3) cur = (double)((count(256, 256) + 255) / 256) * 42;
        else if (tile == 8) cur = (double)((count(192, 256) + 255) / 256) * 38;
        else if (tile == 4) cur = (double)((count(256, 128) + 511) / 512) * 38;
        else cur = count(128, 128) <= 256 ? 16.0 : (double)((count(128, 128) + 511) / 512) * 21;
        int best = 0;
        double bc = 1e30;
        for (int h16 = 9; h16 <= 20; ++h16) {
            const double c = (double)((count(16 * h16, 256) + 255) / 256) * (h16 + 26);
            if (c < bc) bc = c, best = h16;
        }
        if (bc * 100 <= cur * 106) tile = 300 + best;
    }
    if (tile >= 106 && tile <= 110) tile = 300 + 2 * (tile - 100);
    if (tile >= 309 && tile <= 320) {
        VLMO_CHECK_ARG(dtype == VLMO_BF16 && !gp.g[0].k1, "vlmo_gemm_nt: tiles 106..110 / 309..320 are bf16, single-source");
        ProfScope prof(80 + epi, 2.0 * Mtot * N * K, stream);
        return launch_nt16_height(tile - 300, epi, gp, stream);
    }
    VLMO_CHECK_ARG(tile == 0 || tile == 3 || tile == 4 || tile == 8, "vlmo_gemm_nt: tile must be -1, 0, 3, 4, 8, 106..110 or 309..320 (got %d)", tile);
    if (tile == 4 && !(dtype == VLMO_BF16 && (epi == VLMO_EPI_BIAS || epi == VLMO_EPI_BIAS_GELU))) tile = 0;
    if (tile == 8 && !(dtype == VLMO_BF16 && (epi == VLMO_EPI_BIAS || epi == VLMO_EPI_BIAS_GELU || epi == VLMO_EPI_RESID || epi == VLMO_EPI_DGELU))) tile = 3;
    ProfScope prof(epi + (tile == 3 || tile == 8 ? 16 : (tile == 4 ? 48 : 0)), 2.0 * Mtot * N * K, stream);
    if (tile == 4)
        return launch_nt<bf16, 256, 128, 2, 2, false, 32, 2, false, (1u << VLMO_EPI_BIAS) | (1u << VLMO_EPI_BIAS_GELU)>(epi, gp, stream);
    if (tile == 8)
        return launch_nt<bf16, 192, 256, 2, 4, false, 64, 2, true,
                         (1u << VLMO_EPI_BIAS) | (1u << VLMO_EPI_BIAS_GELU) | (1u << VLMO_EPI_RESID) | (1u << VLMO_EPI_DGELU)>(epi, gp, stream);
    if (dtype == VLMO_F16) {
        if (tile == 3) return launch_nt<f16, 256, 256, 2, 4, false, 64, 2, true>(epi, gp, stream);
        return launch_nt<f16, 128, 128, 2, 2>(epi, gp, stream);
    }
    if (tile == 3) return launch_nt<bf16, 256, 256, 2, 4, false, 64, 2, true>(epi, gp, stream);
    return launch_nt<bf16, 128, 128, 2, 2>(epi, gp, stream);
}

int group_m_for(int N, int K) {
    return (long)N * K * 2 <= 5l << 20 ? 1 : 4;
}
}

extern "C" int vlmo_gemm_nt(int epi, int dtype, int tile, const void* A, int lda, const void* B, int ldb,
                            int M, int N, int K, const VlmoEpilogue* e, hipStream_t stream) {
    if (int rc = check_nt(epi, A, lda, B, ldb, M, N, K, e)) return rc;
    GemmNTGroups gp{};
    gp.ngroups = 1;
    gp.g[0] = GemmNT{A, B, M, N, K, lda, ldb, *e, 0, 0, 0, 0, nullptr, group_m_for(N, K), nullptr, 0, 0, 1.f};
    return run_nt(epi, dtype, tile, gp, stream);
}

extern "C" int vlmo_gemm_nt_2src(int epi, int dtype, int tile, const void* A, int lda, int k1, float seg_scale,
                                 const void* A2, int lda2, const void* B, int ldb, int M, int N, int K,
                                 const VlmoEpilogue* e, hipStream_t stream) {
    VLMO_CHECK_ARG(A2 && k1 > 0 && k1 < K && k1 % 64 == 0, "vlmo_gemm_nt_2src: need 0 < k1 < K, k1 %% 64 == 0 (k1=%d, K=%d)", k1, K);
    VLMO_CHECK_ARG(dtype == VLMO_F16, "vlmo_gemm_nt_2src: instantiated for f16 (the dVAE encoder) only");
    VLMO_CHECK_ARG(lda % 8 == 0 && lda >= k1 && lda2 % 8 == 0 && lda2 >= K - k1, "vlmo_gemm_nt_2src: bad lda/lda2 %d/%d", lda, lda2);
    if (int rc = check_nt(epi, A, K > lda ? K : lda, B, ldb, M, N, K, e)) return rc;
    GemmNTGroups gp{};
    gp.ngroups = 1;
    gp.g[0] = GemmNT{A, B, M, N, K, lda, ldb, *e, 0, 0, 0, 0, nullptr, group_m_for(N, K), A2, lda2, k1, seg_scale};
    return run_nt(epi, dtype, tile, gp, stream);
}

extern "C" int vlmo_gemm_nt_grouped(int epi, int dtype, int tile, int ngroups, const void* const* A, int lda,
                                    const void* const* B, int ldb, const int32_t* M, int N, int K,
                                    const VlmoEpilogue* e, hipStream_t stream) {
    VLMO_CHECK_ARG(ngroups >= 1 && ngroups <= MAX_GROUPS && A && B && M && e, "vlmo_gemm_nt_grouped: 1..%d groups", MAX_GROUPS);
    VLMO_CHECK_ARG(epi != VLMO_EPI_ARGMAX && epi != VLMO_EPI_CE, "vlmo_gemm_nt_grouped: the arg-max / cross-entropy epilogues are single-problem");
    GemmNTGroups gp{};
    gp.ngroups = ngroups;
    for (int q = 0; q < ngroups; ++q) {
        if (int rc = check_nt(epi, A[q], lda, B[q], ldb, M[q], N, K, &e[q])) return rc;
        gp.g[q] = GemmNT{A[q], B[q], M[q], N, K, lda, ldb, e[q], 0, 0, 0, 0, nullptr, group_m_for(N, K), nullptr, 0, 0, 1.f};
    }
    return run_nt(epi, dtype, tile, gp, stream);
}
```

### exploremultimodal_amd/csrc/gemm_nt16.hip

```cpp
#include "gemm_common.h"
#include <type_traits>
#include <utility>

namespace {

template <typename T, int EPI> struct ExtRaw { typedef f32x4 type; };
template <typename T> struct ExtRaw<T, VLMO_EPI_DGELU> { typedef typename Elem<T>::v4 type; };
template <typename T, int EPI>
__device__ __forceinline__ typename ExtRaw<T, EPI>::type epilogue_ext_raw(const GemmNT& p, int gmb, int rowc, int gnc) {
    if constexpr (EPI == VLMO_EPI_DGELU) {
        const RowAddr o2{(size_t)gmb * p.e.ld2, (uint32_t)(rowc * p.e.ld2 + gnc)};
        return NT_LD((const typename Elem<T>::v4*)o2.at<T>(p.e.aux));
    } else {
        return epilogue_ext<T, EPI>(p, gmb, rowc, gnc);
    }
}
template <typename T> __device__ __forceinline__ f32x4 ext_f32(f32x4 v) { return v; }
template <typename T> __device__ __forceinline__ f32x4 ext_f32(typename Elem<T>::v4 v) {
    return f32x4{(float)v[0], (float)v[1], (float)v[2], (float)v[3]};
}

template <int... Is, typename F> __device__ __forceinline__ void static_for(std::integer_sequence<int, Is...>, F&& f) {
    (f(std::integral_constant<int, Is>{}), ...);
}

template <typename T, int H16, int EPI, int GD = 0>
__global__ __launch_bounds__(512, 2) void gemm_nt16_kernel(const GemmNTGroups gp) {
    typedef typename Elem<T>::v8 v8;
    constexpr int TMA = (H16 + 1) / 2, TMB = H16 / 2;
    constexpr int BM = 16 * H16, WN = 4, BN = WN * 64, BK = 64, NW = 2 * WN;
    constexpr int ROWB = BK * 2, SRPI = 1024 / ROWB, CPR = ROWB / 16;
    constexpr int A_BYTES = BM * ROWB, B_BYTES = BN * ROWB, STAGE = A_BYTES + B_BYTES;
    constexpr int NAI = BM / SRPI;
    constexpr int NA = (NAI + NW - 1) / NW, NB = BN / SRPI / NW;
    static_assert(NW * 32 * 64 * 4 <= 2 * STAGE, "epilogue LDS must fit in the ring");
    extern __shared__ __attribute__((aligned(16))) char smem[];

    const int tid = threadIdx.x, lane = tid & 63;
    const int wave = __builtin_amdgcn_readfirstlane(tid >> 6);
    const int wm = wave / WN, wn = wave % WN;
    const int la = xcd_remap(blockIdx.x, gridDim.x);
    int gi = 0;
#pragma unroll
    for (int q = 1; q < MAX_GROUPS; ++q)
        if (q < gp.ngroups && la >= gp.t0[q]) gi = q;
    gi = __builtin_amdgcn_readfirstlane(gi);
    GemmNT p;
    {
        const GemmNT& gq = gp.g[gi];
        p.A = uniform_ptr(gq.A), p.B = uniform_ptr(gq.B);
        p.M = uniform_i(gq.M), p.N = uniform_i(gq.N), p.K = uniform_i(gq.K), p.lda = uniform_i(gq.lda), p.ldb = uniform_i(gq.ldb);
        p.group_m = uniform_i(gq.group_m);
        p.e.out = (void*)uniform_ptr(gq.e.out), p.e.out2 = (void*)uniform_ptr(gq.e.out2);
        p.e.bias = (const float*)uniform_ptr(gq.e.bias), p.e.gamma = (const float*)uniform_ptr(gq.e.gamma);
        p.e.resid = (const float*)uniform_ptr(gq.e.resid), p.e.row_scale = (const float*)uniform_ptr(gq.e.row_scale);
        p.e.row_index = (const int32_t*)uniform_ptr(gq.e.row_index), p.e.aux = uniform_ptr(gq.e.aux);
        p.e.ldo = uniform_i(gq.e.ldo), p.e.ld2 = uniform_i(gq.e.ld2), p.e.relu = uniform_i(gq.e.relu);
        p.e.drop_thresh = (uint32_t)uniform_i((int)gq.e.drop_thresh);
        p.e.inv_keep = uniform_f(gq.e.inv_keep), p.e.beta = uniform_f(gq.e.beta);
        p.e.seed = (uint64_t)uniform_ptr((const void*)gq.e.seed);
        p.e.colpart = (float*)uniform_ptr(gq.e.colpart);
    }
    int m0, n0;
    {
        const int tiles_n = (p.N + BN - 1) / BN, tiles_m = (p.M + BM - 1) / BM;
        const int lid = la - uniform_i(gp.t0[gi]);
        const int gm_ = p.group_m > 0 ? p.group_m : 1;
        const int per_group = gm_ * tiles_n;
        const int first_m = (lid / per_group) * gm_;
        const int gsz = min(tiles_m - first_m, gm_);
        const int in_g = lid % per_group;
        m0 = (first_m + in_g % gsz) * BM;
        n0 = (in_g / gsz) * BN;
    }
    const char* a_base = (const char*)p.A + (size_t)m0 * p.lda * 2;
    const char* b_base = (const char*)p.B + (size_t)n0 * p.ldb * 2;
    uint32_t a_off[NA], b_off[NB];
    auto chunk_of = [&](int rr) { return (lane % CPR) ^ nt_swz<64>(rr); };
#pragma unroll
    for (int i = 0; i < NA; ++i) {
        const int rr = (i * NW + wave) * SRPI + lane / CPR;
        const int gr = min(m0 + rr, p.M - 1) - m0;
        a_off[i] = (uint32_t)((gr * p.lda + chunk_of(rr) * 8) * 2);
    }
#pragma unroll
    for (int i = 0; i < NB; ++i) {
        const int rr = (i * NW + wave) * SRPI + lane / CPR;
        const int gr = min(n0 + rr, p.N - 1) - n0;
        b_off[i] = (uint32_t)((gr * p.ldb + chunk_of(rr) * 8) * 2);
    }
    BufSrc a_rs, b_rs;
    a_rs.init(a_base);
    b_rs.init(b_base);
    auto stage = [&](int buf, int kt) {
        char* s = smem + buf * STAGE;
        const int koff = kt * ROWB;
#pragma unroll
        for (int i = 0; i < NA; ++i)
            if ((i + 1) * NW <= NAI || i * NW + wave < NAI)
                a_rs.load16(s + (i * NW + wave) * 1024, a_off[i], koff);
#pragma unroll
        for (int i = 0; i < NB; ++i)
            b_rs.load16(s + A_BYTES + (i * NW + wave) * 1024, b_off[i], koff);
    };

    auto body = [&](auto tm_c, auto row0_c) __attribute__((always_inline)) {
        constexpr int TM = decltype(tm_c)::value, ROW0 = decltype(row0_c)::value;
        f32x4 acc[TM][4];
    #pragma unroll
        for (int i = 0; i < TM; ++i)
    #pragma unroll
            for (int j = 0; j < 4; ++j) acc[i][j] = f32x4{0.f, 0.f, 0.f, 0.f};
        const int l15 = lane & 15, g4 = lane >> 4;
        const int swz = (l15 >> 1) & 7;
        const int a_row_off = (ROW0 + l15) * ROWB;
        const int b_row_off = A_BYTES + (wn * 64 + l15) * ROWB;
        const int nk = p.K / BK;

        stage(0, 0);
        {
            v8 af[TM], bf[4];
            auto read_half = [&](const char* s_, int hf) {
                const int coff = ((4 * hf + g4) ^ swz) << 4;
    #pragma unroll
                for (int j = 0; j < 4; ++j) bf[j] = *(const v8*)(s_ + b_row_off + j * 16 * ROWB + coff);
    #pragma unroll
                for (int i = 0; i < TM; ++i) af[i] = *(const v8*)(s_ + a_row_off + i * 16 * ROWB + coff);
            };
            auto mfma_half = [&]() {
                __builtin_amdgcn_s_setprio(1);
    #pragma unroll
                for (int i = 0; i < TM; ++i)
    #pragma unroll
                    for (int j = 0; j < 4; ++j) acc[i][j] = Elem<T>::mfma16(af[i], bf[j], acc[i][j]);
                __builtin_amdgcn_s_setprio(0);
            };
            auto bar = [&]() {
                __builtin_amdgcn_sched_barrier(0);
                asm volatile("s_waitcnt lgkmcnt(0)" ::: "memory");
                __builtin_amdgcn_s_barrier();
                asm volatile("" ::: "memory");
                __builtin_amdgcn_sched_barrier(0);
            };
            asm volatile("s_waitcnt vmcnt(0)" ::: "memory");
            __builtin_amdgcn_s_barrier();
            if (wm == 1) bar();
            for (int kt = 0; kt < nk; ++kt) {
                const char* cur = smem + (kt & 1) * STAGE;
                const bool more = kt + 1 < nk;
                read_half(cur, 0);
                if (more) stage((kt + 1) & 1, kt + 1);
                bar();
                mfma_half();
                bar();
                read_half(cur, 1);
                if (more && wm == 1) asm volatile("s_waitcnt vmcnt(0)" ::: "memory");
                bar();
                mfma_half();
                if (more && wm == 0) asm volatile("s_waitcnt vmcnt(0)" ::: "memory");
                bar();
            }
            if (wm == 0) bar();
        }

        __syncthreads();
        constexpr int ROWF = 64, LPR = 16, RPI = 4;
        float* ep = (float*)(smem + wave * (32 * ROWF * 4));
        const int rrow = lane / LPR, rcol = (lane % LPR) * 4;
        const int gn = n0 + wn * 64 + rcol;
        const bool col_ok = gn < p.N;
        const int gnc = col_ok ? gn : 0;
        f32x4 bias4 = {0.f, 0.f, 0.f, 0.f}, gamma4 = {1.f, 1.f, 1.f, 1.f};
        if (p.e.bias) bias4 = *(const f32x4*)(p.e.bias + gnc);
        if (EPI == VLMO_EPI_RESID && p.e.gamma) gamma4 = *(const f32x4*)(p.e.gamma + gnc);
        typedef typename ExtRaw<T, EPI>::type XR;
        constexpr int NP = (TM + 1) / 2;
        constexpr bool AHEAD = (EPI == VLMO_EPI_DGELU) || (EPI == VLMO_EPI_RESID && TM <= 7);
        XR xr[2][8];
        float rsv[2][8];
        auto epi_load = [&](auto pi_c) __attribute__((always_inline)) {
            constexpr int P = decltype(pi_c)::value, I0 = 2 * P, NR = (I0 + 2 <= TM) ? 2 : 1;
            constexpr int NIT = NR * 16 / RPI;
            const int gmb = __builtin_amdgcn_readfirstlane(m0 + ROW0 + I0 * 16);
            const int gmbc = min(gmb, p.M - 1);
            int ridx[NIT];
    #pragma unroll
            for (int it = 0; it < NIT; ++it) {
                const int gmc = gmbc + min(it * RPI + rrow, p.M - 1 - gmbc);
                ridx[it] = (EPI == VLMO_EPI_RESID && p.e.row_scale && p.e.row_index) ? p.e.row_index[gmc] : gmc;
            }
    #pragma unroll
            for (int it = 0; it < NIT; ++it) {
                const int rowc = min(it * RPI + rrow, p.M - 1 - gmbc);
                xr[P & 1][it] = epilogue_ext_raw<T, EPI>(p, gmbc, rowc, gnc);
                rsv[P & 1][it] = (EPI == VLMO_EPI_RESID && p.e.row_scale) ? p.e.row_scale[ridx[it]] : 1.f;
            }
        };
        auto epi_pass = [&](auto pi_c) __attribute__((always_inline)) {
            constexpr int P = decltype(pi_c)::value, I0 = 2 * P, NR = (I0 + 2 <= TM) ? 2 : 1;
            constexpr int NIT = NR * 16 / RPI;
            const int gmb = __builtin_amdgcn_readfirstlane(m0 + ROW0 + I0 * 16);
            if constexpr (!AHEAD) epi_load(pi_c);
    #pragma unroll
            for (int ii = 0; ii < NR; ++ii)
    #pragma unroll
                for (int j = 0; j < 4; ++j)
    #pragma unroll
                    for (int r = 0; r < 4; ++r) ep[(ii * 16 + 4 * g4 + r) * ROWF + j * 16 + l15] = acc[I0 + ii][j][r];
            __builtin_amdgcn_fence(__ATOMIC_RELEASE, "wavefront");
            __builtin_amdgcn_wave_barrier();
            __builtin_amdgcn_fence(__ATOMIC_ACQUIRE, "wavefront");
            f32x4 v[NIT];
    #pragma unroll
            for (int it = 0; it < NIT; ++it) v[it] = *(const f32x4*)(ep + (it * RPI + rrow) * ROWF + rcol);
            if constexpr (AHEAD && P + 1 < NP) epi_load(std::integral_constant<int, P + 1>{});
            f32x4 csum = {0.f, 0.f, 0.f, 0.f};
    #pragma unroll
            for (int it = 0; it < NIT; ++it) {
                const int row = it * RPI + rrow;
                const bool ok = gmb + row < p.M && col_ok;
                const f32x4 w = epilogue4<T, EPI, GD>(p, gmb, row, gn, v[it], bias4, gamma4, ext_f32<T>(xr[P & 1][it]), rsv[P & 1][it], ok);
                if constexpr (EPI == VLMO_EPI_DGELU) {
    #pragma unroll
                    for (int j = 0; j < 4; ++j) csum[j] += ok ? w[j] : 0.f;
                }
            }
            __builtin_amdgcn_fence(__ATOMIC_RELEASE, "wavefront");
            __builtin_amdgcn_wave_barrier();
            __builtin_amdgcn_fence(__ATOMIC_ACQUIRE, "wavefront");
            if constexpr (EPI == VLMO_EPI_DGELU) {
                if (p.e.colpart) {
    #pragma unroll
                    for (int o = LPR; o < 64; o <<= 1)
    #pragma unroll
                        for (int j = 0; j < 4; ++j) csum[j] += __shfl_xor(csum[j], o, 64);
                    const int blk = gmb >> 4;
                    if (lane < LPR && col_ok && gmb < p.M) {
                        *(f32x4*)(p.e.colpart + (size_t)blk * p.N + gn) = csum;
                        if (NR == 2 && gmb + 16 < p.M) *(f32x4*)(p.e.colpart + (size_t)(blk + 1) * p.N + gn) = f32x4{0.f, 0.f, 0.f, 0.f};
                    }
                }
            }
        };
        if constexpr (AHEAD) epi_load(std::integral_constant<int, 0>{});
        static_for(std::make_integer_sequence<int, NP>{}, [&](auto pi) __attribute__((always_inline)) {
            epi_pass(std::integral_constant<int, decltype(pi)::value>{});
        });
    };
    if (wm == 0)
        body(std::integral_constant<int, TMA>{}, std::integral_constant<int, 0>{});
    else
        body(std::integral_constant<int, TMB>{}, std::integral_constant<int, 16 * TMA>{});
}

template <typename T, int H16>
int launch_nt16(int epi, GemmNTGroups& p, hipStream_t st) {
    constexpr int BM = 16 * H16, BN = 256, BK = 64;
    int tiles = 0;
    for (int q = 0; q < p.ngroups; ++q) {
        p.t0[q] = tiles;
        tiles += ((p.g[q].M + BM - 1) / BM) * ((p.g[q].N + BN - 1) / BN);
    }
    for (int q = p.ngroups; q <= MAX_GROUPS; ++q) p.t0[q] = tiles;
    constexpr int LDS = 2 * (BM + BN) * BK * 2;
    dim3 grid(tiles), block(512);
    bool known = true;
    const bool gd = (p.g[0].e.relu & 4) != 0;
    for (int q = 1; q < p.ngroups; ++q)
        if (((p.g[q].e.relu & 4) != 0) != gd) {
            vlmo_set_error("vlmo_gemm_nt_grouped: the groups of a launch must agree on VlmoEpilogue.relu bit 2");
            return -1;
        }
#define VLMO_LAUNCH16(E)                                                                        \
    case E: {                                                                                   \
        constexpr bool HAS_GD = (E == VLMO_EPI_BIAS_GELU || E == VLMO_EPI_DGELU);                         \
        if (HAS_GD && gd) {                                                                     \
            auto k = gemm_nt16_kernel<T, H16, E, HAS_GD ? 1 : 0>;                               \
            static DeviceOnce attr_set;                                                         \
            if (LDS > 65536 && attr_set.first())                                                \
                (void)hipFuncSetAttribute((const void*)k, hipFuncAttributeMaxDynamicSharedMemorySize, LDS); \
            hipLaunchKernelGGL(k, grid, block, LDS, st, p);                                     \
        } else {                                                                                \
            auto k = gemm_nt16_kernel<T, H16, E, 0>;                                            \
            static DeviceOnce attr_set;                                                         \
            if (LDS > 65536 && attr_set.first())                                                \
                (void)hipFuncSetAttribute((const void*)k, hipFuncAttributeMaxDynamicSharedMemorySize, LDS); \
            hipLaunchKernelGGL(k, grid, block, LDS, st, p);                                     \
        }                                                                                       \
    } break;
    switch (epi) {
        VLMO_LAUNCH16(VLMO_EPI_BIAS)
        VLMO_LAUNCH16(VLMO_EPI_BIAS_GELU)
        VLMO_LAUNCH16(VLMO_EPI_RESID)
        VLMO_LAUNCH16(VLMO_EPI_DGELU)
        default:
            known = false;
    }
#undef VLMO_LAUNCH16
    if (!known) {
        vlmo_set_error("vlmo_gemm_nt: this 16x16x32 tile is not built with epilogue %d", epi);
        return -1;
    }
    VLMO_CHECK_LAUNCH("vlmo_gemm_nt");
    return 0;
}

}

extern "C" int launch_nt16_height(int h16, int epi, GemmNTGroups& gp, hipStream_t stream) {
    switch (h16) {
        case 9: return launch_nt16<bf16, 9>(epi, gp, stream);
        case 10: return launch_nt16<bf16, 10>(epi, gp, stream);
        case 11: return launch_nt16<bf16, 11>(epi, gp, stream);
        case 12: return launch_nt16<bf16, 12>(epi, gp, stream);
        case 13: return launch_nt16<bf16, 13>(epi, gp, stream);
        case 14: return launch_nt16<bf16, 14>(epi, gp, stream);
        case 15: return launch_nt16<bf16, 15>(epi, gp, stream);
        case 16: return launch_nt16<bf16, 16>(epi, gp, stream);
        case 17: return launch_nt16<bf16, 17>(epi, gp, stream);
        case 18: return launch_nt16<bf16, 18>(epi, gp, stream);
        case 19: return launch_nt16<bf16, 19>(epi, gp, stream);
        default: return launch_nt16<bf16, 20>(epi, gp, stream);
    }
}
```

### exploremultimodal_amd/hip.py

```python
import ctypes
import os

import numpy as np
import torch

_HERE = os.path.dirname(os.path.abspath(__file__))
LIB_PATH = os.environ.get('VLMO_HIP_LIB') or os.path.join(_HERE, 'lib', 'libvlmo_hip.so')

BF16, F16, F32 = 0, 1, 2
EPI_BIAS, EPI_BIAS_GELU, EPI_RESID, EPI_DGELU, EPI_F32, EPI_DUAL, EPI_ARGMAX, EPI_CE, EPI_CE_BWD = 0, 1, 2, 3, 4, 5, 6, 7, 8

_vp, _i32, _u32, _u64, _f32, _i64 = (ctypes.c_void_p, ctypes.c_int32, ctypes.c_uint32,
                                     ctypes.c_uint64, ctypes.c_float, ctypes.c_int64)


class Epilogue(ctypes.Structure):
    _fields_ = [('out', _vp), ('out2', _vp), ('bias', _vp), ('gamma', _vp),
                ('resid', _vp), ('row_scale', _vp), ('row_index', _vp), ('aux', _vp),
                ('ldo', _i32), ('ld2', _i32), ('relu', _i32),
                ('drop_thresh', _u32), ('inv_keep', _f32), ('beta', _f32),
                ('seed', _u64), ('colpart', _vp)]


_fp = _vp


class BlockDesc(ctypes.Structure):
    _fields_ = (
        [('M', _i32), ('d', _i32), ('hidden', _i32), ('heads', _i32),
         ('n_experts', _i32), ('exp_row0', _i32 * 2), ('exp_rows', _i32 * 2),
         ('n_attn', _i32), ('nseq', _i32 * 2), ('maxlen', _i32 * 2), ('lse_stride', _i32 * 2),
         ('attn_seed_idx', _i32 * 2), ('attn_seq0', _i32 * 2),
         ('seg', _fp * 2), ('keymask', _fp), ('eps', _f32),
         ('drop_thresh', _u32), ('attn_drop_thresh', _u32), ('inv_keep', _f32), ('attn_inv_keep', _f32),
         ('seed', _u64), ('rs1', _fp), ('rs2', _fp), ('row_index', _fp), ('tile', _i32), ('need_bwd', _i32)]
        + [(n, _fp) for n in ('g1', 'g2', 'n1w', 'n1b', 'n2w', 'n2b', 'qkv_bias', 'proj_b',
                              'qkv_w', 'qkv_wT', 'proj_w', 'proj_wT')]
        + [(n, _fp * 2) for n in ('b1', 'b2', 'w1', 'w1T', 'w2', 'w2T')]
        + [(n, _fp) for n in ('x', 'x1', 'x2', 'y1', 'qkv', 'ctx', 'zd1', 'y2', 'u', 'h', 'zd2',
                              'mean1', 'rstd1', 'mean2', 'rstd2')]
        + [('lse', _fp * 2)]
        + [(n, _fp) for n in ('dx2', 'dx1', 'dx0', 'dz2', 'du', 'dy2', 'dz1', 'dctx', 'dqkv', 'dy1',
                              'dg1', 'dg2', 'dn1w', 'dn1b', 'dn2w', 'dn2b', 'dqkv_w', 'dqkv_b',
                              'dproj_w', 'dproj_b')]
        + [(n, _fp * 2) for n in ('dw1', 'db1', 'dw2', 'db2')]
        + [('ws_main', _fp), ('ws_bytes', _i64)])


class StackDesc(ctypes.Structure):
    _fields_ = [('n_blocks', _i32), ('wgrad_batch', _i32), ('n_tmp_sets', _i32), ('wgrad_store', _i32),
                ('blocks', ctypes.POINTER(BlockDesc)), ('side_stream', _vp), ('grad_ready', ctypes.POINTER(_vp))]


class TnProblem(ctypes.Structure):
    _fields_ = [('A', _vp), ('B', _vp), ('C', _vp), ('lda', _i32), ('ldb', _i32), ('ldc', _i32),
                ('M', _i32), ('N1', _i32), ('N2', _i32), ('alpha', _f32), ('accumulate', _i32)]


class TnProblemPlan(ctypes.Structure):
    _fields_ = [('tiles', _i32), ('splits', _i32), ('kt_per_split', _i32), ('mode', _i32), ('zero_first', _i32)]


class ColJob(ctypes.Structure):
    _fields_ = [('kind', _i32), ('ld', _i32), ('src', _vp), ('rows', _i32), ('ncols', _i32),
                ('out', _vp * 4), ('n0', _i32), ('pad_', _i32)]


class Image(ctypes.Structure):
    _fields_ = [('offset', _i64), ('H', _i32), ('W', _i32)]


class AugSlot(ctypes.Structure):
    _fields_ = [('op', _i32), ('pad_', _i32), ('a', ctypes.c_double), ('b', ctypes.c_double)]


class CropJob(ctypes.Structure):
    _fields_ = [('image', _i32), ('top', _i32), ('left', _i32), ('h', _i32), ('w', _i32), ('flip', _i32), ('S', _i32),
                ('filter', _i32), ('finish', _i32), ('pad_', _i32), ('tmp_off', _i64), ('out', _vp)]


_SIGS = {
    'vlmo_gemm_nt': [_i32, _i32, _i32, _vp, _i32, _vp, _i32, _i32, _i32, _i32,
                     ctypes.POINTER(Epilogue), _vp],
    'vlmo_gemm_tn': [_i32, _vp, _i32, _vp, _i32, _vp, _i32, _i32, _i32, _i32, _f32, _i32, _vp, _i64, _vp],
    'vlmo_ln_fwd': [_vp, _vp, _vp, _vp, _i32, _vp, _vp, _vp, _i32, _i32, _f32, _vp],
    'vlmo_ln_bwd': [_vp, _i32, _vp, _vp, _vp, _vp, _vp, _vp, _vp, _vp, _vp, _i32, _i32, _vp, _i64, _vp],
    'vlmo_ln_resid_bwd': [_vp, _vp, _vp, _vp, _vp, _vp, _vp, _vp, _vp, _vp, _vp, _vp, _vp, _vp, _vp, _vp, _u32, _f32, _u64,
                          _i32, _i32, _vp, _i64, _vp],
    'vlmo_attn_fwd': [_vp, _vp, _i32, _vp, _vp, _vp, _i32, _i32, _i32, _i32, _f32, _u32, _f32,
                      _u64, _i32, _vp],
    'vlmo_attn_bwd': [_vp, _vp, _vp, _vp, _i32, _vp, _i32, _vp, _vp, _vp, _i32, _i32, _i32, _f32,
                      _u32, _f32, _u64, _i32, _vp],
    'vlmo_attn_probs': [_vp, _vp, _i32, _vp, _vp, _i32, _i32, _i32, _i32, _i32, _i32, _f32, _vp],
    'vlmo_attn_gradcam': [_vp, _vp, _vp, _i32, _vp, _vp, _i32, _i32, _i32, _i32, _i32, _i32, _i32, _f32, _vp],
    'vlmo_resid_bwd': [_vp, _vp, _vp, _vp, _vp, _vp, _vp, _vp, _i32, _i32, _u32, _f32, _u64, _vp, _i64, _vp],
    'vlmo_colsum': [_i32, _vp, _i32, _vp, _i32, _i32, _vp, _i64, _vp],
    'vlmo_cast_weight': [_i32, _vp, _i32, _i32, _vp, _vp, _vp],
    'vlmo_cast_weight_multi': [_i32, _i32, _vp, _vp, _vp, _vp, _vp, _vp],
    'vlmo_patchify': [_vp, _vp, _i32, _i32, _i32, _i32, _i32, _vp],
    'vlmo_embed_img_finish': [_vp, _vp, _vp, _vp, _vp, _vp, _vp, _i32, _i32, _i32, _u32, _f32,
                              _u64, _vp],
    'vlmo_embed_img_bwd': [_vp, _vp, _vp, _vp, _vp, _vp, _vp, _i32, _i32, _i32, _u32, _f32,
                           _u64, _vp],
    'vlmo_embed_txt_fwd': [_vp] * 10 + [_i32, _i32, _i32, _f32, _u32, _f32, _u64, _vp],
    'vlmo_embed_txt_bwd': [_vp] * 11 + [_i32, _i32, _i32, _u32, _f32, _u64, _vp],
    'vlmo_embed_txt_rows_fwd': [_vp] * 11 + [_i32, _i32, _i32, _f32, _u32, _f32, _u64, _vp],
    'vlmo_embed_txt_rows_bwd': [_vp] * 13 + [_i64, _i32, _i32, _i32, _i32, _u32, _f32, _u64, _vp],
    'vlmo_conv2d_nhwc': [_i32, _i32, _vp, _i32, _i32, _i32, _i32, _i32, _vp, _i32, _vp,
                         ctypes.POINTER(Epilogue), _vp],
    'vlmo_dvae_im2col': [_vp, _vp, _i32, _i32, _i32, _i32, _i32, _i32, _vp],
    'vlmo_maxpool2_nhwc': [_vp, _vp, _vp, _i32, _i32, _i32, _i32, _vp],
    'vlmo_argmax_reduce': [_vp, _i32, _vp, _i32, _vp],
    'vlmo_dvae_embed': [_vp, _vp, _vp, _vp, _i32, _i32, _i32, _vp],
    'vlmo_upsample2_nhwc': [_vp, _vp, _i32, _i32, _i32, _i32, _vp],
    'vlmo_dvae_out_head': [_vp, _vp, _vp, _vp, _i32, _i32, _i32, _i32, _i32, _vp],
    'vlmo_conv4s2_nhwc': [_i32, _vp, _i32, _i32, _i32, _i32, _vp, _i32, _vp, ctypes.POINTER(Epilogue), _vp],
    'vlmo_convt4s2_nhwc': [_i32, _vp, _i32, _i32, _i32, _i32, _vp, _i32, _vp, ctypes.POINTER(Epilogue), _vp],
    'vlmo_dvae_patch4s2': [_vp, _vp, _i32, _i32, _i32, _i32, _i32, _vp],
    'vlmo_dvae_out_head_linear': [_vp, _vp, _vp, _vp, _i32, _i32, _i32, _i32, _i32, _vp],
    'vlmo_ce_reduce': [_vp, _i32, _vp, _i32, _vp, _vp, _vp, _i32, _vp],
    'vlmo_stack_fwd': [ctypes.POINTER(StackDesc), _vp],
    'vlmo_stack_bwd': [ctypes.POINTER(StackDesc), _vp],
    'vlmo_gemm_tn_multi': [_i32, ctypes.POINTER(TnProblem), _i32, _vp],
    'vlmo_gemm_tn_multi_plan': [ctypes.POINTER(TnProblem), _i32, ctypes.POINTER(_i32), ctypes.POINTER(_i32),
                                ctypes.POINTER(TnProblemPlan), ctypes.POINTER(_i32), ctypes.POINTER(ctypes.c_uint16)],
    'vlmo_colwork_multi': [_i32, ctypes.POINTER(ColJob), _i32, _vp],
    'vlmo_event_create': [ctypes.POINTER(ctypes.c_void_p)],
    'vlmo_event_destroy': [_vp],
    'vlmo_stream_wait_event': [_vp, _vp],
    'vlmo_profile_start': [_i32],
    'vlmo_gemm_nt_grouped': [_i32, _i32, _i32, _i32, _vp, _i32, _vp, _i32, _vp, _i32, _i32, _vp, _vp],
    'vlmo_mt_grad_norm': [ctypes.c_void_p, _f32, _f32, _vp, _vp, _vp],
    'vlmo_mt_adam': [ctypes.c_void_p, ctypes.c_void_p, _vp, _vp],
    'vlmo_mt_ema': [ctypes.c_void_p, _f32, _vp],
    'vlmo_mt_adam_ema': [ctypes.c_void_p, ctypes.c_void_p, _vp, _vp, _f32, _vp],
    'vlmo_side_stream_create': [_i32, ctypes.POINTER(ctypes.c_uint32), _i32, ctypes.POINTER(ctypes.c_void_p)],
    'vlmo_profile_stop': [_i32, ctypes.POINTER(ctypes.c_double), ctypes.POINTER(ctypes.c_double),
                          ctypes.POINTER(ctypes.c_int64)],
    'vlmo_gemm_nt_2src': [_i32, _i32, _i32, _vp, _i32, _i32, _f32, _vp, _i32, _vp, _i32, _i32, _i32, _i32,
                          ctypes.POINTER(Epilogue), _vp],
    'vlmo_comm_available': [],
    'vlmo_comm_unique_id': [_vp],
    'vlmo_comm_init': [ctypes.POINTER(ctypes.c_void_p), _vp, _i32, _i32],
    'vlmo_comm_destroy': [_vp],
    'vlmo_comm_count': [_vp, _vp, _vp],
    'vlmo_comm_all_reduce': [_vp, _vp, _vp, _i64, _i32, _vp],
    'vlmo_comm_reduce_scatter': [_vp, _vp, _vp, _i64, _i32, _vp],
    'vlmo_comm_all_gather': [_vp, _vp, _vp, _i64, _i32, _vp],
    'vlmo_grad_pack': [_vp, _vp, _i64, _f32, _vp],
    'vlmo_grad_unpack': [_vp, _vp, _i64, _vp],
    'vlmo_ln_gelu_fwd': [_vp, _i32, _vp, _vp, _vp, _i32, _vp, _vp, _i32, _i32, _f32, _vp],
    'vlmo_ln_gelu_bwd': [_vp, _i32, _vp, _i32, _vp, _vp, _vp, _vp, _vp, _i32, _vp, _i32, _vp, _vp, _vp, _i32, _i32, _vp,
                         _i64, _vp],
    'vlmo_vqa_bce': [_vp, _i32, _vp, _i32, _i32, _i32, _vp, _vp, _vp, _vp, _f32, _vp, _i32, _vp, _i32, _vp],
    'vlmo_isda_update': [_vp, _i32, _vp, _vp, _vp, _vp, _vp, _i32, _i32, _i32, _i32, _vp, _vp, _vp, _vp, _vp],
    'vlmo_isda_aug_fwd': [_vp, _i32, _vp, _vp, _i32, _i32, _i32, _i32, _f32, _vp, _i32, _vp, _i64, _vp],
    'vlmo_isda_aug_bwd': [_vp, _i32, _vp, _i32, _vp, _vp, _i32, _i32, _i32, _i32, _f32, _vp, _i32, _vp, _i64, _vp],
    'vlmo_sim_topk': [_vp, _i32, _vp, _i32, _i32, _i32, _i32, _i32, _f32, _i32, _vp, ctypes.c_size_t, _vp, _vp, _vp],
    'vlmo_crop_resample': [_vp, _i64, _vp, _vp, _i32, _vp, _vp, _i32, ctypes.POINTER(_f32), ctypes.POINTER(_f32), _f32, _vp,
                           _i64, _vp],
    'vlmo_randaug': [_vp, _vp, _vp, _i64, _vp, _vp, _i32, _vp, _vp, _i32, _i32, _vp, _i64, _vp],
}

_lib = None
ABI_VERSION = 16

def lib():
    global _lib
    if _lib is None:
        if not os.path.exists(LIB_PATH):
            raise RuntimeError(
                f'{LIB_PATH} not found: build the HIP extension first '
                '(python -c "import __graft_entry__ as g; g.build()" or '
                'make -C exploremultimodal_amd/csrc). There is no CPU fallback.')
        L = ctypes.CDLL(LIB_PATH)
        L.vlmo_last_error.restype = ctypes.c_char_p
        L.vlmo_abi_version.restype = ctypes.c_int
        if L.vlmo_abi_version() != ABI_VERSION:
            raise RuntimeError(f'{LIB_PATH} has ABI version {L.vlmo_abi_version()}, this package needs {ABI_VERSION}: '
                               'rebuild it (make -C exploremultimodal_amd/csrc)')
        L.vlmo_reduce_ws_bytes.restype = ctypes.c_int64
        L.vlmo_reduce_ws_bytes.argtypes = [_i32]
        L.vlmo_stack_bwd_ws_bytes.restype = ctypes.c_int64
        L.vlmo_stack_bwd_ws_bytes.argtypes = [_i32, _i32, _i32, _i32]
        L.vlmo_gemm_tn_ws_bytes.restype = ctypes.c_int64
        L.vlmo_isda_ws_bytes.restype = ctypes.c_int64
        L.vlmo_isda_ws_bytes.argtypes = [_i32, _i32, _i32]
        L.vlmo_gemm_tn_ws_bytes.argtypes = [_i32, _i32, _i32]
        L.vlmo_sim_topk_ws_bytes.restype = ctypes.c_int64
        L.vlmo_sim_topk_ws_bytes.argtypes = [_i32, _i32, _i32, _i32]
        L.vlmo_randaug_ws_bytes.restype = ctypes.c_int64
        L.vlmo_randaug_ws_bytes.argtypes = [_i32]
        L.vlmo_embed_txt_rows_ws_bytes.restype = ctypes.c_int64
        L.vlmo_embed_txt_rows_ws_bytes.argtypes = [_i32, _i32, _i32]
        for name, sig in _SIGS.items():
            fn = getattr(L, name)
            fn.argtypes = sig
            fn.restype = ctypes.c_int
        _lib = L
    return _lib


def exported_symbols():
    return ['vlmo_last_error', 'vlmo_abi_version', 'vlmo_reduce_ws_bytes', 'vlmo_stack_bwd_ws_bytes',
            'vlmo_gemm_tn_ws_bytes', 'vlmo_isda_ws_bytes', 'vlmo_sim_topk_ws_bytes', 'vlmo_randaug_ws_bytes',
            'vlmo_embed_txt_rows_ws_bytes'] + list(_SIGS)


def _check(rc, name):
    if rc != 0:
        raise RuntimeError(f'{name} failed (rc={rc}): {lib().vlmo_last_error().decode()}')


def _p(t):
    return None if t is None else t.data_ptr()


def _stream():
    return torch.cuda.current_stream().cuda_stream


def _dt(t):
    return {torch.bfloat16: BF16, torch.float16: F16, torch.float32: F32}[t.dtype]


_SCRATCH = {}


def _scratch(kind, device, nbytes, floor):
    key = (kind, device, torch.cuda.current_stream(device).cuda_stream)
    ws = _SCRATCH.get(key)
    if ws is None or ws.numel() * 4 < nbytes:
        ws = torch.empty(max(nbytes, floor) // 4, dtype=torch.float32, device=device)
        _SCRATCH[key] = ws
    return ws


def workspace(device, ncols):
    return _scratch('reduce', device, lib().vlmo_reduce_ws_bytes(ncols), 1 << 23)


def tn_workspace(device, nbytes):
    return _scratch('tn', device, nbytes, 1 << 24)


def drop_params(p, training):
    if not training or p <= 0.0:
        return 0, 1.0
    thresh = int(round(p * 65536))
    return thresh, 65536.0 / (65536 - thresh)


def _seed64(seed):
    return seed & 0xFFFFFFFFFFFFFFFF


def _epilogue(out, *, out2=None, bias=None, gamma=None, resid=None, row_scale=None, row_index=None, aux=None, ldo=None,
              ld2=None, relu=False, drop=(0, 1.0), seed=0, beta=0.0, colpart=None):
    if ld2 is None:
        ld2 = out2.stride(0) if out2 is not None else (aux.stride(0) if aux is not None else 0)
    return Epilogue(_p(out), _p(out2), _p(bias), _p(gamma), _p(resid), _p(row_scale), _p(row_index), _p(aux),
                    ldo if ldo is not None else out.stride(0), ld2, int(relu), drop[0], drop[1], beta, _seed64(seed),
                    _p(colpart))



def gemm_nt(epi, A, B, M, N, K, out, *, tile=-1, lda=None, ldb=None, A2=None, k1=0, seg_scale=1.0, **epilogue):
    e = _epilogue(out, **epilogue)
    if A2 is not None:
        rc = lib().vlmo_gemm_nt_2src(epi, _dt(A), tile, _p(A), lda if lda is not None else A.stride(0), k1,
                                     float(seg_scale), _p(A2), A2.stride(0), _p(B),
                                     ldb if ldb is not None else B.stride(0), M, N, K, ctypes.byref(e), _stream())
        _check(rc, 'vlmo_gemm_nt_2src')
        return
    rc = lib().vlmo_gemm_nt(epi, _dt(A), tile, _p(A), lda if lda is not None else A.stride(0),
                            _p(B), ldb if ldb is not None else B.stride(0), M, N, K,
                            ctypes.byref(e), _stream())
    _check(rc, 'vlmo_gemm_nt')


def gemm_nt_grouped(epi, As, Bs, Ms, N, K, outs, *, per_group=None, tile=-1, **common):
    n = len(As)
    es = (Epilogue * n)()
    for g in range(n):
        es[g] = _epilogue(outs[g], **{**common, **(per_group[g] if per_group else {})})
    pa = (ctypes.c_void_p * n)(*[_p(a) for a in As])
    pb = (ctypes.c_void_p * n)(*[_p(b) for b in Bs])
    ms = (ctypes.c_int32 * n)(*Ms)
    rc = lib().vlmo_gemm_nt_grouped(epi, _dt(As[0]), tile, n, pa, As[0].stride(0), pb, Bs[0].stride(0), ms, N, K, es, _stream())
    _check(rc, 'vlmo_gemm_nt_grouped')


def gemm_tn(A, B, C, M, N1, N2, alpha=1.0, splits=0, slab=True):
    ws = tn_workspace(A.device, max(splits % 1000, 16) * N1 * N2 * 4 if splits > 0 else
                      lib().vlmo_gemm_tn_ws_bytes(M, N1, N2)) if slab else None
    rc = lib().vlmo_gemm_tn(_dt(A), _p(A), A.stride(0), _p(B), B.stride(0), _p(C), C.stride(0),
                            M, N1, N2, alpha, splits, _p(ws), ws.numel() * 4 if ws is not None else 0, _stream())
    _check(rc, 'vlmo_gemm_tn')


def ln_fwd(x, w, b, y, mean, rstd, rowmap, M, d, eps):
    rc = lib().vlmo_ln_fwd(_p(x), _p(w), _p(b), _p(y), int(y.dtype == torch.float32), _p(mean),
                           _p(rstd), _p(rowmap), M, d, eps, _stream())
    _check(rc, 'vlmo_ln_fwd')


def ln_bwd(dy, rowmap, x, w, mean, rstd, dres, dx, dw, db, M, d):
    rc = lib().vlmo_ln_bwd(_p(dy), int(dy.dtype == torch.float32), _p(rowmap), _p(x), _p(w),
                           _p(mean), _p(rstd), _p(dres), _p(dx), _p(dw), _p(db), M, d, _p(ws := workspace(x.device, 2 * d)),
                           ws.numel() * 4, _stream())
    _check(rc, 'vlmo_ln_bwd')


def ln_resid_bwd(dy, x, w, mean, rstd, dres, dx, dw, db, zd, gamma, row_scale, row_index, dz, dgamma, dbias, M, d,
                 drop=(0, 1.0), seed=0):
    ws = workspace(x.device, 4 * d)
    rc = lib().vlmo_ln_resid_bwd(_p(dy), _p(x), _p(w), _p(mean), _p(rstd), _p(dres), _p(dx), _p(dw), _p(db), _p(zd),
                                 _p(gamma), _p(row_scale), _p(row_index), _p(dz), _p(dgamma), _p(dbias), drop[0], drop[1],
                                 _seed64(seed), M, d, _p(ws), ws.numel() * 4, _stream())
    _check(rc, 'vlmo_ln_resid_bwd')


def attn_fwd(qkv, seg, nseq, keymask, ctx, lse, heads, d, max_len, scale, drop=(0, 1.0), seed=0, mask_seq0=0):
    rc = lib().vlmo_attn_fwd(_p(qkv), _p(seg), nseq, _p(keymask), _p(ctx), _p(lse),
                             lse.stride(0) if lse is not None else 0, heads, d, max_len, scale,
                             drop[0], drop[1], _seed64(seed), mask_seq0, _stream())
    _check(rc, 'vlmo_attn_fwd')


def attn_bwd(qkv, ctx, dctx, lse, seg, nseq, keymask, dqkv, heads, d, max_len, scale,
             drop=(0, 1.0), seed=0, qv_colsum=None, mask_seq0=0):
    rc = lib().vlmo_attn_bwd(_p(qkv), _p(ctx), _p(dctx), _p(lse), lse.stride(0), _p(seg), nseq,
                             _p(keymask), _p(dqkv), _p(qv_colsum), heads, d, max_len, scale, drop[0], drop[1],
                             _seed64(seed), mask_seq0, _stream())
    _check(rc, 'vlmo_attn_bwd')


def attn_probs(qkv, seg, nseq, keymask, probs, heads, d, seq_len, q0, nq, head_mean, scale):
    rc = lib().vlmo_attn_probs(_p(qkv), _p(seg), nseq, _p(keymask), _p(probs), heads, d, seq_len, q0, nq,
                               int(bool(head_mean)), scale, _stream())
    _check(rc, 'vlmo_attn_probs')


GRADCAM_KINDS = {'cam': 0, 'attn_grad': 1, 'grad': 2}


def attn_gradcam(qkv, dctx, seg, nseq, keymask, out, heads, d, seq_len, q0, nq, kind, head_mean, scale):
    rc = lib().vlmo_attn_gradcam(_p(qkv), _p(dctx), _p(seg), nseq, _p(keymask), _p(out), heads, d, seq_len, q0, nq,
                                 GRADCAM_KINDS.get(kind, kind), int(bool(head_mean)), scale, _stream())
    _check(rc, 'vlmo_attn_gradcam')


def resid_bwd(dx, zd, gamma, row_scale, dz, dgamma, dbias, M, d, drop=(0, 1.0), seed=0, row_index=None):
    ws = workspace(dx.device, 2 * d)
    rc = lib().vlmo_resid_bwd(_p(dx), _p(zd), _p(gamma), _p(row_scale), _p(row_index), _p(dz), _p(dgamma),
                              _p(dbias), M, d, drop[0], drop[1], _seed64(seed),
                              _p(ws), ws.numel() * 4, _stream())
    _check(rc, 'vlmo_resid_bwd')


def colsum(x, out, M, N):
    ws = workspace(x.device, N)
    rc = lib().vlmo_colsum(_dt(x), _p(x), x.stride(0), _p(out), M, N, _p(ws), ws.numel() * 4, _stream())
    _check(rc, 'vlmo_colsum')


def cast_weight(src, dst, dstT):
    rows, cols = src.shape
    ref = dst if dst is not None else dstT
    rc = lib().vlmo_cast_weight(_dt(ref), _p(src), rows, cols, _p(dst), _p(dstT), _stream())
    _check(rc, 'vlmo_cast_weight')


def cast_weight_multi(jobs):
    n = len(jobs)
    if n == 0:
        return
    ref = jobs[0][1] if jobs[0][1] is not None else jobs[0][2]
    src = (ctypes.c_void_p * n)(*[_p(a) for a, _, _ in jobs])
    dst = (ctypes.c_void_p * n)(*[_p(b) for _, b, _ in jobs])
    dstT = (ctypes.c_void_p * n)(*[_p(c) for _, _, c in jobs])
    rows = (ctypes.c_int32 * n)(*[a.shape[0] for a, _, _ in jobs])
    cols = (ctypes.c_int32 * n)(*[a.shape[1] for a, _, _ in jobs])
    _check(lib().vlmo_cast_weight_multi(_dt(ref), n, src, rows, cols, dst, dstT, _stream()), 'vlmo_cast_weight_multi')


def patchify(img, out, patch):
    B, C, H, W = img.shape
    rc = lib().vlmo_patchify(_p(img), _p(out), B, C, H, W, patch, _stream())
    _check(rc, 'vlmo_patchify')


def embed_img_finish(proj, cls_tok, mask_tok, pos, type_row, masked, x, B, npatch, d,
                     drop=(0, 1.0), seed=0):
    rc = lib().vlmo_embed_img_finish(_p(proj), _p(cls_tok), _p(mask_tok), _p(pos), _p(type_row),
                                     _p(masked), _p(x), B, npatch, d, drop[0], drop[1],
                                     _seed64(seed), _stream())
    _check(rc, 'vlmo_embed_img_finish')


def embed_img_bwd(dx, masked, dproj, dcls, dmask, dpos, dtype_row, B, npatch, d, drop=(0, 1.0),
                  seed=0):
    rc = lib().vlmo_embed_img_bwd(_p(dx), _p(masked), _p(dproj), _p(dcls), _p(dmask), _p(dpos),
                                  _p(dtype_row), B, npatch, d, drop[0], drop[1],
                                  _seed64(seed), _stream())
    _check(rc, 'vlmo_embed_img_bwd')


def embed_txt_fwd(ids, word, pos, btype0, ln_w, ln_b, type0, x, xhat, rstd, B, T, d, eps,
                  drop=(0, 1.0), seed=0):
    rc = lib().vlmo_embed_txt_fwd(_p(ids), _p(word), _p(pos), _p(btype0), _p(ln_w), _p(ln_b),
                                  _p(type0), _p(x), _p(xhat), _p(rstd), B, T, d, eps, drop[0],
                                  drop[1], _seed64(seed), _stream())
    _check(rc, 'vlmo_embed_txt_fwd')
# ... 325 lines not shown
    m3, s3 = (_f32 * 3)(*mean), (_f32 * 3)(*std)
    _check(lib().vlmo_crop_resample(_p(pixels), pixels.numel(), ih, idev, len(itab), jh, jdev, len(jtab), m3, s3,
                                    float(pixel_eps), _p(ws), ws.numel() * 4, _stream()), 'vlmo_crop_resample')


(AUG_SKIP, AUG_IDENTITY, AUG_AUTOCONTRAST, AUG_EQUALIZE, AUG_BRIGHTNESS, AUG_SHARPNESS, AUG_SHEAR_X, AUG_SHEAR_Y,
 AUG_TRANSLATE_X, AUG_TRANSLATE_Y, AUG_ROTATE, AUG_SOLARIZE, AUG_POSTERIZE, AUG_CONTRAST) = range(-1, 13)
AUG_MAX_SLOTS, AUG_MAX_IMAGES, AUG_MAX_SHIFT = 4, 65536, 1000000


def randaug(pixels, images, ops, a, b, fill=128, out=None, scratch=None, ws=None):
    ops = np.asarray(ops, dtype=np.int64)
    a, b = np.asarray(a, dtype=np.float64), np.asarray(b, dtype=np.float64)
    ni = len(images)
    if ops.ndim != 2 or ops.shape[0] != ni or a.shape != ops.shape or b.shape != ops.shape:
        raise ValueError(f'randaug: ops, a and b must be [{ni}, n] (got {ops.shape}, {a.shape}, {b.shape})')
    n = ops.shape[1]
    if out is None:
        out = torch.empty_like(pixels)
    if scratch is None and n > 1:
        scratch = torch.empty_like(pixels)
    for t, name in ((pixels, 'pixels'), (out, 'out'), (scratch, 'scratch')):
        if t is not None and (t.dtype != torch.uint8 or t.dim() != 1 or not t.is_contiguous() or t.device != pixels.device
                              or t.numel() != pixels.numel()):
            raise ValueError(f'randaug: {name} must be a contiguous 1-D uint8 buffer of pixels\' length and device')
    if ws is None:
        ws = _scratch('randaug', pixels.device, lib().vlmo_randaug_ws_bytes(ni), 1 << 20)
    (ih, idev, sh, sdev), keep = _stage_tables(pixels.device, image_records(images), aug_slot_records(ops, a, b))
    _check(lib().vlmo_randaug(_p(pixels), _p(out), _p(scratch), pixels.numel(), ih, idev, ni, sh, sdev, n, int(fill), _p(ws),
                              ws.numel() * ws.element_size(), _stream()), 'vlmo_randaug')
    return out


PROFILE_TAGS = 96


class TensorList(ctypes.Structure):
    _fields_ = [('p', _vp), ('g', _vp), ('m', _vp), ('v', _vp), ('numel', _vp), ('lr', _vp), ('wd', _vp),
                ('chunk_tensor', _vp), ('chunk_start', _vp), ('n_chunks', _i32), ('chunk', _i32)]


class AdamArgs(ctypes.Structure):
    _fields_ = [('beta1', _f32), ('beta2', _f32), ('eps', _f32), ('inv_bc1', _f32), ('inv_bc2', _f32),
                ('adam_w_mode', _i32)]


def mt_grad_norm(tl, inv_scale, max_norm, partial, out):
    _check(lib().vlmo_mt_grad_norm(ctypes.byref(tl), float(inv_scale), float(max_norm), _p(partial), _p(out), _stream()),
           'vlmo_mt_grad_norm')


def mt_adam(tl, args, ctl=None):
    _check(lib().vlmo_mt_adam(ctypes.byref(tl), ctypes.byref(args), _p(ctl), _stream()), 'vlmo_mt_adam')


def mt_ema(tl, w):
    _check(lib().vlmo_mt_ema(ctypes.byref(tl), float(w), _stream()), 'vlmo_mt_ema')


def mt_adam_ema(tl, args, ctl, ema, w):
    _check(lib().vlmo_mt_adam_ema(ctypes.byref(tl), ctypes.byref(args), _p(ctl), _p(ema), float(w), _stream()),
           'vlmo_mt_adam_ema')


def side_stream_create(low_priority=True, cu_mask=None):
    out = ctypes.c_void_p()
    if cu_mask:
        words = (ctypes.c_uint32 * len(cu_mask))(*cu_mask)
        rc = lib().vlmo_side_stream_create(0, words, len(cu_mask), ctypes.byref(out))
    else:
        rc = lib().vlmo_side_stream_create(1 if low_priority else 0, None, 0, ctypes.byref(out))
    _check(rc, 'vlmo_side_stream_create')
    return out.value


def profile_start(max_records=1 << 15):
    _check(lib().vlmo_profile_start(max_records), 'vlmo_profile_start')


def profile_stop():
    n = PROFILE_TAGS
    ms, fl, ln = (ctypes.c_double * n)(), (ctypes.c_double * n)(), (ctypes.c_int64 * n)()
    lib().vlmo_profile_stop(n, ms, fl, ln)
    names = {0: 'bias', 1: 'bias_gelu', 2: 'resid', 3: 'dgelu', 4: 'f32', 5: 'dual', 6: 'argmax', 7: 'ce', 8: 'ce_bwd'}
    out = {}
    for t in range(n):
        if ln[t]:
            if t in (64, 72):
                name = 'gemm_tn_kernel<%s>' % ('256x256' if t == 72 else '128x128')
            elif t == 73:
                name = 'gemm_tn_multi_kernel<256x256>'
            elif 80 <= t < 96:
                name = f'gemm_nt16_kernel<{names.get(t - 80, t - 80)},Hx256>'
            elif 48 <= t < 64:
                name = f'gemm_nt_kernel<{names.get(t - 48, t - 48)},256x128>'
            elif t >= 32:
                name = f'conv_nt_kernel<{names.get(t - 32, t - 32)}>'
            else:
                name = f'gemm_nt_kernel<{names.get(t & 15, t & 15)},{"256x256" if t & 16 else "128x128"}>'
            out[name] = (ms[t] * 1e-3, fl[t], ln[t])
    return out
```

### include/vlmo_hip.h

```cpp
#ifndef VLMO_HIP_H
#define VLMO_HIP_H

#include <stddef.h>
#include <stdint.h>

#ifdef __cplusplus
extern "C" {
#endif

#ifndef __HIP_PLATFORM_AMD__
typedef struct ihipStream_t* hipStream_t;
#endif

enum { VLMO_BF16 = 0, VLMO_F16 = 1, VLMO_F32 = 2 };

enum {
    VLMO_EPI_BIAS = 0,
    VLMO_EPI_BIAS_GELU = 1,
    VLMO_EPI_RESID = 2,
    VLMO_EPI_DGELU = 3,
    VLMO_EPI_F32 = 4,
    VLMO_EPI_DUAL = 5,
    VLMO_EPI_ARGMAX = 6,
    VLMO_EPI_CE = 7,
    VLMO_EPI_CE_BWD = 8
};

typedef struct VlmoEpilogue {
    void* out;
    void* out2;
    const float* bias;
    const float* gamma;
    const float* resid;
    const float* row_scale;
    const int32_t* row_index;
    const void* aux;
    int32_t ldo, ld2;
    int32_t relu;
    uint32_t drop_thresh;
    float inv_keep;
    float beta;
    uint64_t seed;
    float* colpart;
} VlmoEpilogue;

const char* vlmo_last_error(void);
#define VLMO_ABI_VERSION 16
int vlmo_abi_version(void);

int vlmo_gemm_nt(int epi, int dtype, int tile, const void* A, int lda, const void* B, int ldb,
                 int M, int N, int K, const VlmoEpilogue* e, hipStream_t stream);
int vlmo_gemm_nt_2src(int epi, int dtype, int tile, const void* A, int lda, int k1, float seg_scale, const void* A2,
                      int lda2, const void* B, int ldb, int M, int N, int K, const VlmoEpilogue* e,
                      hipStream_t stream);
int vlmo_gemm_nt_grouped(int epi, int dtype, int tile, int ngroups, const void* const* A, int lda,
                         const void* const* B, int ldb, const int32_t* M, int N, int K,
                         const VlmoEpilogue* e, hipStream_t stream);

int64_t vlmo_gemm_tn_ws_bytes(int M, int N1, int N2);
int vlmo_gemm_tn(int dtype, const void* A, int lda, const void* B, int ldb, float* C, int ldc,
                 int M, int N1, int N2, float alpha, int splits, float* ws, int64_t ws_bytes,
                 hipStream_t stream);

typedef struct VlmoTnProblem {
    const void* A;
    const void* B;
    float* C;
    int32_t lda, ldb, ldc;
    int32_t M, N1, N2;
    float alpha;
    int32_t accumulate;
} VlmoTnProblem;
int vlmo_gemm_tn_multi(int dtype, const VlmoTnProblem* probs, int n, hipStream_t stream);
typedef struct VlmoTnProblemPlan {
    int32_t tiles;
    int32_t splits;
    int32_t kt_per_split;
    int32_t mode;
    int32_t zero_first;
} VlmoTnProblemPlan;
int vlmo_gemm_tn_multi_plan(const VlmoTnProblem* probs, int n, int32_t* n_launches, int32_t* launch_q0,
                            VlmoTnProblemPlan* prob, int32_t* grid, uint16_t* order);

int vlmo_ln_fwd(const float* x, const float* w, const float* b, void* y, int out_f32,
                float* mean, float* rstd, const int32_t* rowmap, int M, int d, float eps,
                hipStream_t stream);
int64_t vlmo_reduce_ws_bytes(int ncols);

int vlmo_ln_bwd(const void* dy, int dy_f32, const int32_t* rowmap, const float* x, const float* w,
                const float* mean, const float* rstd, const float* dres, float* dx, float* dw,
                float* db, int M, int d, float* ws, int64_t ws_bytes, hipStream_t stream);

int vlmo_ln_resid_bwd(const void* dy, const float* x, const float* w, const float* mean, const float* rstd,
                      const float* dres, float* dx, float* dw, float* db, const void* zd, const float* gamma,
                      const float* row_scale, const int32_t* row_index, void* dz, float* dgamma, float* dbias,
                      uint32_t drop_thresh, float inv_keep, uint64_t seed, int M, int d, float* ws,
                      int64_t ws_bytes, hipStream_t stream);

int vlmo_attn_fwd(const void* qkv, const int32_t* seg, int num_seq, const int32_t* keymask,
                  void* ctx, float* lse, int lse_stride, int heads, int d, int max_len,
                  float scale, uint32_t drop_thresh, float inv_keep, uint64_t seed, int mask_seq0,
                  hipStream_t stream);
int vlmo_attn_bwd(const void* qkv, const void* ctx, const void* dctx, const float* lse,
                  int lse_stride, const int32_t* seg, int num_seq, const int32_t* keymask,
                  void* dqkv, float* qv_colsum, int heads, int d, int max_len, float scale,
                  uint32_t drop_thresh, float inv_keep, uint64_t seed, int mask_seq0, hipStream_t stream);

int vlmo_attn_probs(const void* qkv, const int32_t* seg, int num_seq, const int32_t* keymask, float* probs,
                    int heads, int d, int seq_len, int q0, int nq, int head_mean, float scale, hipStream_t stream);

#define VLMO_GRADCAM_CAM 0
#define VLMO_GRADCAM_ATTN_GRAD 1
#define VLMO_GRADCAM_GRAD 2
int vlmo_attn_gradcam(const void* qkv, const void* dctx, const int32_t* seg, int num_seq, const int32_t* keymask,
                      float* out, int heads, int d, int seq_len, int q0, int nq, int kind, int head_mean, float scale,
                      hipStream_t stream);

int vlmo_resid_bwd(const float* dx, const void* zd, const float* gamma, const float* row_scale,
                   const int32_t* row_index, void* dz, float* dgamma, float* dbias, int M, int d,
                   uint32_t drop_thresh,
                   float inv_keep, uint64_t seed, float* ws, int64_t ws_bytes, hipStream_t stream);

int vlmo_colsum(int dtype, const void* x, int ld, float* out, int M, int N, float* ws,
                int64_t ws_bytes, hipStream_t stream);

typedef struct VlmoColJob {
    int32_t kind, ld;
    const void* src;
    int32_t rows, ncols;
    float* out[4];
    int32_t n0, pad_;
} VlmoColJob;
int vlmo_colwork_multi(int dtype, const VlmoColJob* jobs, int n, hipStream_t stream);

int vlmo_cast_weight(int dtype, const float* src, int rows, int cols, void* dst, void* dstT,
                     hipStream_t stream);
int vlmo_cast_weight_multi(int dtype, int n, const float* const* src, const int32_t* rows, const int32_t* cols,
                           void* const* dst, void* const* dstT, hipStream_t stream);

int vlmo_patchify(const float* img, void* out, int B, int C, int H, int W, int patch,
                  hipStream_t stream);
int vlmo_embed_img_finish(const void* proj, const float* cls_tok, const float* mask_tok,
                          const float* pos, const float* type_row, const uint8_t* masked_pos,
                          float* x, int B, int npatch, int d, uint32_t drop_thresh,
                          float inv_keep, uint64_t seed, hipStream_t stream);
int vlmo_embed_img_bwd(const float* dx, const uint8_t* masked_pos, void* dproj, float* dcls,
                       float* dmask, float* dpos, float* dtype_row, int B, int npatch, int d,
                       uint32_t drop_thresh, float inv_keep, uint64_t seed, hipStream_t stream);

int vlmo_embed_txt_fwd(const int64_t* ids, const float* word, const float* pos, const float* btype0,
                       const float* ln_w, const float* ln_b, const float* type0, float* x,
                       float* xhat, float* rstd, int B, int T, int d, float eps,
                       uint32_t drop_thresh, float inv_keep, uint64_t seed, hipStream_t stream);
int vlmo_embed_txt_bwd(const float* dx, const int64_t* ids, const float* xhat, const float* rstd,
                       const float* ln_w, float* dword, float* dpos, float* dbtype0, float* dln_w,
                       float* dln_b, float* dtype0, int B, int T, int d, uint32_t drop_thresh,
                       float inv_keep, uint64_t seed, hipStream_t stream);
int vlmo_embed_txt_rows_fwd(const int64_t* ids, const int32_t* src, const float* word, const float* pos,
                            const float* btype0, const float* ln_w, const float* ln_b, const float* type0,
                            float* x, float* xhat, float* rstd, int nrows, int T, int d, float eps,
                            uint32_t drop_thresh, float inv_keep, uint64_t seed, hipStream_t stream);
int64_t vlmo_embed_txt_rows_ws_bytes(int B, int maxlen, int d);
int vlmo_embed_txt_rows_bwd(const float* dx, const int64_t* ids, const int32_t* off, const float* xhat,
                            const float* rstd, const float* ln_w, float* dword, float* dpos, float* dbtype0,
                            float* dln_w, float* dln_b, float* dtype0, float* ws, int64_t ws_bytes, int B, int T,
                            int maxlen, int d, uint32_t drop_thresh, float inv_keep, uint64_t seed,
                            hipStream_t stream);

int vlmo_profile_start(int max_records);
int vlmo_profile_stop(int ntags, double* ms, double* flops, int64_t* launches);

typedef struct {
    const int64_t* p;
    const int64_t* g;
    const int64_t* m;
    const int64_t* v;
    const int64_t* numel;
    const float* lr;
    const float* wd;
    const int32_t* chunk_tensor;
    const int64_t* chunk_start;
    int32_t n_chunks, chunk;
} VlmoTensorList;

typedef struct {
    float beta1, beta2, eps;
    float inv_bc1, inv_bc2;
    int32_t adam_w_mode;
} VlmoAdamArgs;
// ... 181 lines not shown
```

Before: 4496.

## Fuse attention-backward row dots into the proj dgrad GEMM epilogue

Measured after the change: 4500 (median of 5 runs). About the same (+0.1%).

```diff
diff --git a/exploremultimodal_amd/csrc/attention.hip b/exploremultimodal_amd/csrc/attention.hip
--- a/exploremultimodal_amd/csrc/attention.hip
+++ b/exploremultimodal_amd/csrc/attention.hip
@@ -7,6 +7,8 @@
     const bf16* qkv;
     const bf16* ctx;
     const bf16* dctx;
+    const float* rowdot;
+    int rowdot_ld;
     bf16* out;
     float* lse;
     float* qvsum;
@@ -550,18 +552,22 @@
         const int row = sr.row(i);
         const float kb = key_bias(a.keymask, row, i, N);
         if (i < N) {
-            const size_t o = (size_t)row * a.d + hd * 64;
-            bf16x8 x[8], y[8];
-#pragma unroll
-            for (int c = 0; c < 8; ++c) {
-                x[c] = *(const bf16x8*)(a.ctx + o + 8 * c);
-                y[c] = *(const bf16x8*)(a.dctx + o + 8 * c);
-            }
             lq = a.lse[(size_t)bh * a.lse_stride + i];
-#pragma unroll
-            for (int c = 0; c < 8; ++c)
-#pragma unroll
-                for (int j = 0; j < 8; ++j) dl += (float)x[c][j] * (float)y[c][j];
+            if (a.rowdot) {
+                dl = a.rowdot[(size_t)hd * a.rowdot_ld + row];
+            } else {
+                const size_t o = (size_t)row * a.d + hd * 64;
+                bf16x8 x[8], y[8];
+#pragma unroll
+                for (int c = 0; c < 8; ++c) {
+                    x[c] = *(const bf16x8*)(a.ctx + o + 8 * c);
+                    y[c] = *(const bf16x8*)(a.dctx + o + 8 * c);
+                }
+#pragma unroll
+                for (int c = 0; c < 8; ++c)
+#pragma unroll
+                    for (int j = 0; j < 8; ++j) dl += (float)x[c][j] * (float)y[c][j];
+            }
         }
         kbias[i] = kb;
         ndl[i] = -dl * keep_prob;
@@ -903,18 +909,22 @@
         float dl = 0.f, lq = INFINITY;
         const int row = sr.row(i);
         if (i < sr.N) {
-            const size_t o = (size_t)row * a.d + hd * 64;
-            bf16x8 x[8], y[8];
-#pragma unroll
-            for (int c = 0; c < 8; ++c) {
-                x[c] = *(const bf16x8*)(a.ctx + o + 8 * c);
-                y[c] = *(const bf16x8*)(a.dctx + o + 8 * c);
-            }
             lq = a.lse[(size_t)bh * a.lse_stride + i] * LOG2E;
-#pragma unroll
-            for (int c = 0; c < 8; ++c)
-#pragma unroll
-                for (int j = 0; j < 8; ++j) dl += (float)x[c][j] * (float)y[c][j];
+            if (a.rowdot) {
+                dl = a.rowdot[(size_t)hd * a.rowdot_ld + row];
+            } else {
+                const size_t o = (size_t)row * a.d + hd * 64;
+                bf16x8 x[8], y[8];
+#pragma unroll
+                for (int c = 0; c < 8; ++c) {
+                    x[c] = *(const bf16x8*)(a.ctx + o + 8 * c);
+                    y[c] = *(const bf16x8*)(a.dctx + o + 8 * c);
+                }
+#pragma unroll
+                for (int c = 0; c < 8; ++c)
+#pragma unroll
+                    for (int j = 0; j < 8; ++j) dl += (float)x[c][j] * (float)y[c][j];
+            }
         }
         delta[i] = dl * keep_prob;
         lseq[i] = lq;
@@ -1567,28 +1577,50 @@
     return 0;
 }
 
-extern "C" int vlmo_attn_bwd(const void* qkv, const void* ctx, const void* dctx, const float* lse, int lse_stride,
-                             const int32_t* seg, int num_seq, const int32_t* keymask, void* dqkv, float* qv_colsum,
-                             int heads, int d, int max_len, float scale, uint32_t drop_thresh, float inv_keep,
-                             uint64_t seed, int mask_seq0, hipStream_t stream) {
-    if (int rc = check_common("vlmo_attn_bwd", qkv, seg, num_seq, heads, d, max_len, 1024)) return rc;
-    VLMO_CHECK_ARG(ctx && dctx && lse && dqkv, "vlmo_attn_bwd: null pointer");
-    VLMO_CHECK_ARG(lse_stride >= max_len, "vlmo_attn_bwd: lse_stride too small");
+namespace {
+int run_bwd(const char* fn, const void* qkv, const void* ctx, const void* dctx, const float* lse, int lse_stride,
+            const int32_t* seg, int num_seq, const int32_t* keymask, void* dqkv, float* qv_colsum, int heads, int d,
+            int max_len, float scale, uint32_t drop_thresh, float inv_keep, uint64_t seed, int mask_seq0,
+            const float* rowdot, int rowdot_ld, hipStream_t stream) {
+    if (int rc = check_common(fn, qkv, seg, num_seq, heads, d, max_len, 1024)) return rc;
+    VLMO_CHECK_ARG((ctx || rowdot) && dctx && lse && dqkv, "%s: null pointer", fn);
+    VLMO_CHECK_ARG(lse_stride >= max_len, "%s: lse_stride too small", fn);
     AttnArgs a = make_args(qkv, seg, keymask, lse, lse_stride, heads, d, scale, drop_thresh, inv_keep, seed, mask_seq0);
     a.ctx = (const bf16*)ctx;
     a.dctx = (const bf16*)dctx;
+    a.rowdot = rowdot;
+    a.rowdot_ld = rowdot_ld;
     a.out = (bf16*)dqkv;
     a.qvsum = qv_colsum;
     const int nt = (max_len + 31) / 32, nb = num_seq * heads;
     if (max_len > 288) {
         launch_bwd_long(a, nb, stream);
-        VLMO_CHECK_LAUNCH("vlmo_attn_bwd(long)");
+        VLMO_CHECK_LAUNCH(fn);
         return 0;
     }
     const int rc = nt > 8 ? launch_bwd1<true>(a, nt, nb, stream) : launch_bwd1<false>(a, nt, nb, stream);
-    VLMO_CHECK_ARG(rc == 0, "vlmo_attn_bwd: %d tokens do not fit the LDS of one CU", max_len);
-    VLMO_CHECK_LAUNCH("vlmo_attn_bwd");
+    VLMO_CHECK_ARG(rc == 0, "%s: %d tokens do not fit the LDS of one CU", fn, max_len);
+    VLMO_CHECK_LAUNCH(fn);
     return 0;
+}
+}
+
+extern "C" int vlmo_attn_bwd(const void* qkv, const void* ctx, const void* dctx, const float* lse, int lse_stride,
+                             const int32_t* seg, int num_seq, const int32_t* keymask, void* dqkv, float* qv_colsum,
+                             int heads, int d, int max_len, float scale, uint32_t drop_thresh, float inv_keep,
+                             uint64_t seed, int mask_seq0, hipStream_t stream) {
+    VLMO_CHECK_ARG(ctx, "vlmo_attn_bwd: null pointer");
+    return run_bwd("vlmo_attn_bwd", qkv, ctx, dctx, lse, lse_stride, seg, num_seq, keymask, dqkv, qv_colsum, heads, d, max_len,
+                   scale, drop_thresh, inv_keep, seed, mask_seq0, nullptr, 0, stream);
+}
+
+extern "C" int vlmo_attn_bwd_rowdot(const void* qkv, const void* ctx, const void* dctx, const float* lse, int lse_stride,
+                                    const int32_t* seg, int num_seq, const int32_t* keymask, void* dqkv, float* qv_colsum,
+                                    int heads, int d, int max_len, float scale, uint32_t drop_thresh, float inv_keep,
+                                    uint64_t seed, int mask_seq0, const float* rowdot, int rowdot_ld, hipStream_t stream) {
+    VLMO_CHECK_ARG(rowdot && rowdot_ld > 0, "vlmo_attn_bwd_rowdot: null rowdot or rowdot_ld <= 0");
+    return run_bwd("vlmo_attn_bwd_rowdot", qkv, ctx, dctx, lse, lse_stride, seg, num_seq, keymask, dqkv, qv_colsum, heads, d,
+                   max_len, scale, drop_thresh, inv_keep, seed, mask_seq0, rowdot, rowdot_ld, stream);
 }
 
 extern "C" int vlmo_attn_probs(const void* qkv, const int32_t* seg, int num_seq, const int32_t* keymask, float* probs,
diff --git a/exploremultimodal_amd/csrc/block.hip b/exploremultimodal_amd/csrc/block.hip
--- a/exploremultimodal_amd/csrc/block.hip
+++ b/exploremultimodal_amd/csrc/block.hip
@@ -175,7 +175,8 @@
 }
 
 int check_block_bwd(const VlmoBlockDesc* b, int i) {
-    VLMO_CHECK_ARG(b->dx2 && b->dx1 && b->dx0, "vlmo_stack_bwd: block %d: null gradient buffers", i);
+    VLMO_CHECK_ARG(b->dx2 && b->dx1 && b->dx0 && b->dy1 && b->ctx, "vlmo_stack_bwd: block %d: null gradient buffers", i);
+    VLMO_CHECK_ARG(b->d == 64 * b->heads, "vlmo_stack_bwd: block %d: head_dim must be 64 (the row dots of the proj dgrad live in dy1)", i);
     VLMO_CHECK_ARG(b->n_experts >= 1 && b->n_experts <= 2 && b->n_attn >= 1 && b->n_attn <= 2,
                    "vlmo_stack_bwd: block %d: 1..2 experts and attention launches per block", i);
     VLMO_CHECK_ARG(b->M > 0 && b->exp_rows[0] >= 0 && (b->n_experts == 1 || b->exp_rows[1] >= 0) &&
@@ -245,18 +246,23 @@
                         2 * slot_bytes, &fold, st));
         push_col(D, fold);
     }
+    float* const rowdot = (float*)b->dy1;
     {
         VlmoEpilogue e = epi();
         e.out = b->dctx;
         e.ldo = d;
-        TRY(vlmo_gemm_nt(VLMO_EPI_BIAS, VLMO_BF16, b->tile, b->dz1, d, b->proj_wT, d, M, d, d, &e, st));
+        e.aux = b->ctx;
+        e.ld2 = d;
+        e.colpart = rowdot;
+        e.ldr = M;
+        TRY(vlmo_gemm_nt(VLMO_EPI_BIAS_ROWDOT, VLMO_BF16, b->tile, b->dz1, d, b->proj_wT, d, M, d, d, &e, st));
     }
     const float scale = 1.0f / sqrtf((float)(d / b->heads));
     float* const qvsum = ws + W.qv;
     for (int a = 0, s0 = 0; a < b->n_attn; s0 += b->nseq[a], ++a)
-        TRY(vlmo_attn_bwd(b->qkv, b->ctx, b->dctx, b->lse[a], b->lse_stride[a], b->seg[a], b->nseq[a], b->keymask,
-                          b->dqkv, qvsum + (size_t)s0 * 2 * d, b->heads, d, b->maxlen[a], scale, b->attn_drop_thresh,
-                          b->attn_inv_keep, b->seed + 11 + b->attn_seed_idx[a], b->attn_seq0[a], st));
+        TRY(vlmo_attn_bwd_rowdot(b->qkv, b->ctx, b->dctx, b->lse[a], b->lse_stride[a], b->seg[a], b->nseq[a], b->keymask,
+                                 b->dqkv, qvsum + (size_t)s0 * 2 * d, b->heads, d, b->maxlen[a], scale, b->attn_drop_thresh,
+                                 b->attn_inv_keep, b->seed + 11 + b->attn_seed_idx[a], b->attn_seq0[a], rowdot, M, st));
     push_tn(D, b->dz1, d, b->ctx, d, b->dproj_w, d, M, d, d);
     push_tn(D, b->dqkv, 3 * d, b->y1, d, b->dqkv_w, d, M, 3 * d, d);
     push_col(D, fold_job(qvsum, 2 * d, nseq_all, 2 * d, d, b->dqkv_b, b->dqkv_b + 2 * d));
diff --git a/exploremultimodal_amd/csrc/common.h b/exploremultimodal_amd/csrc/common.h
--- a/exploremultimodal_amd/csrc/common.h
+++ b/exploremultimodal_amd/csrc/common.h
@@ -190,6 +190,13 @@
     s += dpp_mov<0x143, 0xc, 0xf>(s);
     return __builtin_bit_cast(float, __builtin_amdgcn_readlane(__builtin_bit_cast(int, s), 63));
 }
+__device__ __forceinline__ float row16_sum(float v) {
+    v += dpp_mov<0xB1, 0xf, 0xf>(v);
+    v += dpp_mov<0x4E, 0xf, 0xf>(v);
+    v += dpp_mov<0x141, 0xf, 0xf>(v);
+    v += dpp_mov<0x140, 0xf, 0xf>(v);
+    return v;
+}
 __device__ __forceinline__ float wave_max(float v) {
 #pragma unroll
     for (int o = 32; o > 0; o >>= 1) v = fmaxf(v, __shfl_xor(v, o, 64));
diff --git a/exploremultimodal_amd/csrc/gemm_common.h b/exploremultimodal_amd/csrc/gemm_common.h
--- a/exploremultimodal_amd/csrc/gemm_common.h
+++ b/exploremultimodal_amd/csrc/gemm_common.h
@@ -62,7 +62,7 @@
     const int gm = gmb + row;
     const RowAddr o{(size_t)gmb * e.ldo, (uint32_t)(row * e.ldo + gn)};
     const RowAddr o2{(size_t)gmb * e.ld2, (uint32_t)(row * e.ld2 + gn)};
-    if constexpr (EPI == VLMO_EPI_BIAS) {
+    if constexpr (EPI == VLMO_EPI_BIAS || EPI == VLMO_EPI_BIAS_ROWDOT) {
         const float lo = (e.relu & 1) ? 0.f : -INFINITY;
 #pragma unroll
         for (int j = 0; j < 4; ++j) v[j] = fmaxf(v[j], lo);
@@ -162,7 +162,7 @@
     const RowAddr o2{(size_t)gmb * e.ld2, (uint32_t)(rowc * e.ld2 + gnc)};
     if constexpr (EPI == VLMO_EPI_RESID) {
         return NT_LD((const f32x4*)o.at<float>(e.resid));
-    } else if constexpr (EPI == VLMO_EPI_DGELU) {
+    } else if constexpr (EPI == VLMO_EPI_DGELU || EPI == VLMO_EPI_BIAS_ROWDOT) {
         return load4<T>(o2.at<T>(e.aux));
     } else if constexpr (EPI == VLMO_EPI_DUAL) {
         return e.resid ? load4<T>(o.at<T>(e.resid)) : z;
@@ -171,6 +171,17 @@
     } else {
         return z;
     }
+}
+
+template <typename T> __device__ __forceinline__ float rowdot_lane(f32x4 w, f32x4 x) {
+    float s = (float)(T)w[0] * x[0];
+    s = fmaf((float)(T)w[1], x[1], s);
+    s = fmaf((float)(T)w[2], x[2], s);
+    return fmaf((float)(T)w[3], x[3], s);
+}
+__device__ __forceinline__ void rowdot_store(const GemmNT& p, float s, int lane, int gn, int gm, bool ok) {
+    s = row16_sum(s);
+    if ((lane & 15) == 0 && ok) p.e.colpart[(size_t)(gn >> 6) * (size_t)p.e.ldr + gm] = s;
 }
 
 __device__ __forceinline__ const void* uniform_ptr(const void* p) {
@@ -463,6 +474,7 @@
     __syncthreads();
     constexpr int ROWF = TN * 32;
     constexpr int LPR = TN * 8, RPI = 64 / LPR;
+    static_assert(EPI != VLMO_EPI_BIAS_ROWDOT || LPR == 16, "row dots: a wave's row segment is one 64-column chunk");
     float* ep = (float*)(smem + wave * (32 * ROWF * 4));
     const int rrow = lane / LPR, rcol = (lane % LPR) * 4;
     const int gn = n0 + wn * (BN / WN) + rcol;
@@ -581,6 +593,7 @@
 #pragma unroll
                     for (int j = 0; j < 4; ++j) csum[j] += ok ? w[j] : 0.f;
                 }
+                if constexpr (EPI == VLMO_EPI_BIAS_ROWDOT) rowdot_store(p, rowdot_lane<T>(w, ext[it]), lane, gn, gm, ok);
             }
         }
         __builtin_amdgcn_fence(__ATOMIC_RELEASE, "wavefront");
@@ -614,9 +627,10 @@
     for (int q = p.ngroups; q <= MAX_GROUPS; ++q) p.t0[q] = tiles;
     constexpr int LDS = NSTG * (BM + BN) * BK * 2;
     dim3 grid(tiles), block(WM * WN * 64);
+    constexpr unsigned EM = __is_same(T, bf16) ? EMASK : EMASK & ~(1u << VLMO_EPI_BIAS_ROWDOT);
 #define VLMO_LAUNCH_EPI(E)                                                                     \
     case E:                                                                                    \
-    if constexpr (((EMASK >> E) & 1u) == 0) {                                                  \
+    if constexpr (((EM >> E) & 1u) == 0) {                                                     \
         known = false;                                                                         \
     } else {                                                                                   \
         auto k = gemm_nt_kernel<T, BM, BN, WM, WN, E, CONV, BK, NSTG, PP>;                                        \
@@ -641,6 +655,7 @@
                     VLMO_LAUNCH_EPI(VLMO_EPI_ARGMAX)
                     VLMO_LAUNCH_EPI(VLMO_EPI_CE)
                     VLMO_LAUNCH_EPI(VLMO_EPI_CE_BWD)
+                    VLMO_LAUNCH_EPI(VLMO_EPI_BIAS_ROWDOT)
                     default:
                         known = false;
                 }
diff --git a/exploremultimodal_amd/csrc/gemm_nt.hip b/exploremultimodal_amd/csrc/gemm_nt.hip
--- a/exploremultimodal_amd/csrc/gemm_nt.hip
+++ b/exploremultimodal_amd/csrc/gemm_nt.hip
@@ -78,11 +78,16 @@
     VLMO_CHECK_ARG(epi != VLMO_EPI_ARGMAX || e->ldo >= (N + 63) / 64, "vlmo_gemm_nt: argmax partial buffer too narrow");
     VLMO_CHECK_ARG(epi != VLMO_EPI_RESID || e->resid, "vlmo_gemm_nt: residual epilogue needs resid");
     VLMO_CHECK_ARG(epi != VLMO_EPI_DGELU || (e->aux && e->ld2 >= N), "vlmo_gemm_nt: dgelu epilogue needs aux");
+    VLMO_CHECK_ARG(epi != VLMO_EPI_BIAS_ROWDOT || N % 64 == 0, "vlmo_gemm_nt: row-dot epilogue: N=%d must be a multiple of 64", N);
+    VLMO_CHECK_ARG(epi != VLMO_EPI_BIAS_ROWDOT || (e->aux && e->ld2 >= N && e->ld2 % 4 == 0), "vlmo_gemm_nt: row-dot epilogue needs aux with ld2 >= N, ld2 %% 4 == 0");
+    VLMO_CHECK_ARG(epi != VLMO_EPI_BIAS_ROWDOT || (e->colpart && e->ldr >= M), "vlmo_gemm_nt: row-dot epilogue needs a destination (colpart) with ldr >= M");
     return 0;
 }
 
 int run_nt(int epi, int dtype, int tile, GemmNTGroups& gp, hipStream_t stream) {
     VLMO_CHECK_ARG(dtype == VLMO_BF16 || dtype == VLMO_F16, "vlmo_gemm_nt: dtype must be bf16 or f16");
+    VLMO_CHECK_ARG(epi != VLMO_EPI_BIAS_ROWDOT || dtype == VLMO_BF16, "vlmo_gemm_nt: the row-dot epilogue is bf16");
+    const bool bias_like = epi == VLMO_EPI_BIAS || epi == VLMO_EPI_BIAS_ROWDOT;
     const int tile_in = tile;
     long Mtot = 0;
     for (int q = 0; q < gp.ngroups; ++q) Mtot += gp.g[q].M;
@@ -98,9 +103,9 @@
         for (int q = 0; q < gp.ngroups; ++q) t256_all += (long)((gp.g[q].M + 255) / 256) * ((N + 255) / 256);
         const bool few_tiles = t256_all <= 128;
         if (few_tiles) tile = 0;
-        if (tile == 0 && dtype == VLMO_BF16 && (epi == VLMO_EPI_BIAS || epi == VLMO_EPI_BIAS_GELU) && K <= 1024 && N >= 2048 && Mtot >= 4096)
+        if (tile == 0 && dtype == VLMO_BF16 && (bias_like || epi == VLMO_EPI_BIAS_GELU) && K <= 1024 && N >= 2048 && Mtot >= 4096)
             tile = 4;
-        if (!few_tiles && dtype == VLMO_BF16 && (epi == VLMO_EPI_BIAS || epi == VLMO_EPI_BIAS_GELU || epi == VLMO_EPI_RESID || epi == VLMO_EPI_DGELU) && K >= 1024) {
+        if (!few_tiles && dtype == VLMO_BF16 && (bias_like || epi == VLMO_EPI_BIAS_GELU || epi == VLMO_EPI_RESID || epi == VLMO_EPI_DGELU) && K >= 1024) {
             long t256 = 0, t192n = 0;
             for (int q = 0; q < gp.ngroups; ++q) {
                 t256 += (long)((gp.g[q].M + 255) / 256) * ((N + 255) / 256);
@@ -111,7 +116,7 @@
         }
     }
     if ((tile == 0 || tile == 3 || tile == 4 || tile == 8) && dtype == VLMO_BF16 && !gp.g[0].k1 && !gp.g[0].ckw &&
-        (epi == VLMO_EPI_BIAS || epi == VLMO_EPI_BIAS_GELU || epi == VLMO_EPI_RESID || epi == VLMO_EPI_DGELU) && N >= 512 && K >= 512 &&
+        (bias_like || epi == VLMO_EPI_BIAS_GELU || epi == VLMO_EPI_RESID || epi == VLMO_EPI_DGELU) && N >= 512 && K >= 512 &&
         Mtot * (long)N >= 40 * 65536l && tile_in < 0) {
         auto count = [&](int bm, int bn) {
             long t = 0;
@@ -138,14 +143,15 @@
         return launch_nt16_height(tile - 300, epi, gp, stream);
     }
     VLMO_CHECK_ARG(tile == 0 || tile == 3 || tile == 4 || tile == 8, "vlmo_gemm_nt: tile must be -1, 0, 3, 4, 8, 106..110 or 309..320 (got %d)", tile);
-    if (tile == 4 && !(dtype == VLMO_BF16 && (epi == VLMO_EPI_BIAS || epi == VLMO_EPI_BIAS_GELU))) tile = 0;
-    if (tile == 8 && !(dtype == VLMO_BF16 && (epi == VLMO_EPI_BIAS || epi == VLMO_EPI_BIAS_GELU || epi == VLMO_EPI_RESID || epi == VLMO_EPI_DGELU))) tile = 3;
+    if (tile == 4 && !(dtype == VLMO_BF16 && (bias_like || epi == VLMO_EPI_BIAS_GELU))) tile = 0;
+    if (tile == 8 && !(dtype == VLMO_BF16 && (bias_like || epi == VLMO_EPI_BIAS_GELU || epi == VLMO_EPI_RESID || epi == VLMO_EPI_DGELU))) tile = 3;
     ProfScope prof(epi + (tile == 3 || tile == 8 ? 16 : (tile == 4 ? 48 : 0)), 2.0 * Mtot * N * K, stream);
     if (tile == 4)
-        return launch_nt<bf16, 256, 128, 2, 2, false, 32, 2, false, (1u << VLMO_EPI_BIAS) | (1u << VLMO_EPI_BIAS_GELU)>(epi, gp, stream);
+        return launch_nt<bf16, 256, 128, 2, 2, false, 32, 2, false, (1u << VLMO_EPI_BIAS) | (1u << VLMO_EPI_BIAS_GELU) | (1u << VLMO_EPI_BIAS_ROWDOT)>(epi, gp, stream);
     if (tile == 8)
         return launch_nt<bf16, 192, 256, 2, 4, false, 64, 2, true,
-                         (1u << VLMO_EPI_BIAS) | (1u << VLMO_EPI_BIAS_GELU) | (1u << VLMO_EPI_RESID) | (1u << VLMO_EPI_DGELU)>(epi, gp, stream);
+                         (1u << VLMO_EPI_BIAS) | (1u << VLMO_EPI_BIAS_GELU) | (1u << VLMO_EPI_RESID) | (1u << VLMO_EPI_DGELU) |
+                             (1u << VLMO_EPI_BIAS_ROWDOT)>(epi, gp, stream);
     if (dtype == VLMO_F16) {
         if (tile == 3) return launch_nt<f16, 256, 256, 2, 4, false, 64, 2, true>(epi, gp, stream);
         return launch_nt<f16, 128, 128, 2, 2>(epi, gp, stream);
diff --git a/exploremultimodal_amd/csrc/gemm_nt16.hip b/exploremultimodal_amd/csrc/gemm_nt16.hip
--- a/exploremultimodal_amd/csrc/gemm_nt16.hip
+++ b/exploremultimodal_amd/csrc/gemm_nt16.hip
@@ -6,9 +6,10 @@
 
 template <typename T, int EPI> struct ExtRaw { typedef f32x4 type; };
 template <typename T> struct ExtRaw<T, VLMO_EPI_DGELU> { typedef typename Elem<T>::v4 type; };
+template <typename T> struct ExtRaw<T, VLMO_EPI_BIAS_ROWDOT> { typedef typename Elem<T>::v4 type; };
 template <typename T, int EPI>
 __device__ __forceinline__ typename ExtRaw<T, EPI>::type epilogue_ext_raw(const GemmNT& p, int gmb, int rowc, int gnc) {
-    if constexpr (EPI == VLMO_EPI_DGELU) {
+    if constexpr (EPI == VLMO_EPI_DGELU || EPI == VLMO_EPI_BIAS_ROWDOT) {
         const RowAddr o2{(size_t)gmb * p.e.ld2, (uint32_t)(rowc * p.e.ld2 + gnc)};
         return NT_LD((const typename Elem<T>::v4*)o2.at<T>(p.e.aux));
     } else {
@@ -175,7 +176,7 @@
         if (EPI == VLMO_EPI_RESID && p.e.gamma) gamma4 = *(const f32x4*)(p.e.gamma + gnc);
         typedef typename ExtRaw<T, EPI>::type XR;
         constexpr int NP = (TM + 1) / 2;
-        constexpr bool AHEAD = (EPI == VLMO_EPI_DGELU) || (EPI == VLMO_EPI_RESID && TM <= 7);
+        constexpr bool AHEAD = (EPI == VLMO_EPI_DGELU) || (EPI == VLMO_EPI_BIAS_ROWDOT) || (EPI == VLMO_EPI_RESID && TM <= 7);
         XR xr[2][8];
         float rsv[2][8];
         auto epi_load = [&](auto pi_c) __attribute__((always_inline)) {
@@ -219,7 +220,9 @@
             for (int it = 0; it < NIT; ++it) {
                 const int row = it * RPI + rrow;
                 const bool ok = gmb + row < p.M && col_ok;
-                const f32x4 w = epilogue4<T, EPI, GD>(p, gmb, row, gn, v[it], bias4, gamma4, ext_f32<T>(xr[P & 1][it]), rsv[P & 1][it], ok);
+                const f32x4 x = ext_f32<T>(xr[P & 1][it]);
+                const f32x4 w = epilogue4<T, EPI, GD>(p, gmb, row, gn, v[it], bias4, gamma4, x, rsv[P & 1][it], ok);
+                if constexpr (EPI == VLMO_EPI_BIAS_ROWDOT) rowdot_store(p, rowdot_lane<T>(w, x), lane, gn, gmb + row, ok);
                 if constexpr (EPI == VLMO_EPI_DGELU) {
     #pragma unroll
                     for (int j = 0; j < 4; ++j) csum[j] += ok ? w[j] : 0.f;
@@ -293,6 +296,7 @@
         VLMO_LAUNCH16(VLMO_EPI_BIAS_GELU)
         VLMO_LAUNCH16(VLMO_EPI_RESID)
         VLMO_LAUNCH16(VLMO_EPI_DGELU)
+        VLMO_LAUNCH16(VLMO_EPI_BIAS_ROWDOT)
         default:
             known = false;
     }
diff --git a/exploremultimodal_amd/hip.py b/exploremultimodal_amd/hip.py
--- a/exploremultimodal_amd/hip.py
+++ b/exploremultimodal_amd/hip.py
@@ -8,7 +8,7 @@
 LIB_PATH = os.environ.get('VLMO_HIP_LIB') or os.path.join(_HERE, 'lib', 'libvlmo_hip.so')
 
 BF16, F16, F32 = 0, 1, 2
-EPI_BIAS, EPI_BIAS_GELU, EPI_RESID, EPI_DGELU, EPI_F32, EPI_DUAL, EPI_ARGMAX, EPI_CE, EPI_CE_BWD = 0, 1, 2, 3, 4, 5, 6, 7, 8
+EPI_BIAS, EPI_BIAS_GELU, EPI_RESID, EPI_DGELU, EPI_F32, EPI_DUAL, EPI_ARGMAX, EPI_CE, EPI_CE_BWD, EPI_BIAS_ROWDOT = range(10)
 
 _vp, _i32, _u32, _u64, _f32, _i64 = (ctypes.c_void_p, ctypes.c_int32, ctypes.c_uint32,
                                      ctypes.c_uint64, ctypes.c_float, ctypes.c_int64)
@@ -91,6 +91,8 @@
                       _u64, _i32, _vp],
     'vlmo_attn_bwd': [_vp, _vp, _vp, _vp, _i32, _vp, _i32, _vp, _vp, _vp, _i32, _i32, _i32, _f32,
                       _u32, _f32, _u64, _i32, _vp],
+    'vlmo_attn_bwd_rowdot': [_vp, _vp, _vp, _vp, _i32, _vp, _i32, _vp, _vp, _vp, _i32, _i32, _i32, _f32,
+                             _u32, _f32, _u64, _i32, _vp, _i32, _vp],
     'vlmo_attn_probs': [_vp, _vp, _i32, _vp, _vp, _i32, _i32, _i32, _i32, _i32, _i32, _f32, _vp],
     'vlmo_attn_gradcam': [_vp, _vp, _vp, _i32, _vp, _vp, _i32, _i32, _i32, _i32, _i32, _i32, _i32, _f32, _vp],
     'vlmo_resid_bwd': [_vp, _vp, _vp, _vp, _vp, _vp, _vp, _vp, _i32, _i32, _u32, _f32, _u64, _vp, _i64, _vp],
@@ -163,7 +165,7 @@
 }
 
 _lib = None
-ABI_VERSION = 16
+ABI_VERSION = 17
 
 def lib():
     global _lib
@@ -256,12 +258,12 @@
 
 
 def _epilogue(out, *, out2=None, bias=None, gamma=None, resid=None, row_scale=None, row_index=None, aux=None, ldo=None,
-              ld2=None, relu=False, drop=(0, 1.0), seed=0, beta=0.0, colpart=None):
+              ld2=None, relu=False, drop=(0, 1.0), seed=0, beta=0.0, colpart=None, ldr=0):
     if ld2 is None:
         ld2 = out2.stride(0) if out2 is not None else (aux.stride(0) if aux is not None else 0)
     return Epilogue(_p(out), _p(out2), _p(bias), _p(gamma), _p(resid), _p(row_scale), _p(row_index), _p(aux),
-                    ldo if ldo is not None else out.stride(0), ld2, int(relu), drop[0], drop[1], beta, _seed64(seed),
-                    _p(colpart))
+                    ldo if ldo is not None else out.stride(0), ld2, int(relu), drop[0], drop[1], beta,
+                    _seed64(ldr if ldr else seed), _p(colpart))
 
 
 
@@ -329,7 +331,14 @@
 
 
 def attn_bwd(qkv, ctx, dctx, lse, seg, nseq, keymask, dqkv, heads, d, max_len, scale,
-             drop=(0, 1.0), seed=0, qv_colsum=None, mask_seq0=0):
+             drop=(0, 1.0), seed=0, qv_colsum=None, mask_seq0=0, rowdot=None, rowdot_ld=None):
+    if rowdot is not None:
+        rc = lib().vlmo_attn_bwd_rowdot(_p(qkv), _p(ctx), _p(dctx), _p(lse), lse.stride(0), _p(seg), nseq,
+                                        _p(keymask), _p(dqkv), _p(qv_colsum), heads, d, max_len, scale, drop[0], drop[1],
+                                        _seed64(seed), mask_seq0, _p(rowdot),
+                                        rowdot_ld if rowdot_ld is not None else rowdot.stride(0), _stream())
+        _check(rc, 'vlmo_attn_bwd_rowdot')
+        return
     rc = lib().vlmo_attn_bwd(_p(qkv), _p(ctx), _p(dctx), _p(lse), lse.stride(0), _p(seg), nseq,
                              _p(keymask), _p(dqkv), _p(qv_colsum), heads, d, max_len, scale, drop[0], drop[1],
                              _seed64(seed), mask_seq0, _stream())
@@ -821,7 +830,8 @@
     n = PROFILE_TAGS
     ms, fl, ln = (ctypes.c_double * n)(), (ctypes.c_double * n)(), (ctypes.c_int64 * n)()
     lib().vlmo_profile_stop(n, ms, fl, ln)
-    names = {0: 'bias', 1: 'bias_gelu', 2: 'resid', 3: 'dgelu', 4: 'f32', 5: 'dual', 6: 'argmax', 7: 'ce', 8: 'ce_bwd'}
+    names = {0: 'bias', 1: 'bias_gelu', 2: 'resid', 3: 'dgelu', 4: 'f32', 5: 'dual', 6: 'argmax', 7: 'ce', 8: 'ce_bwd',
+             9: 'bias_rowdot'}
     out = {}
     for t in range(n):
         if ln[t]:
diff --git a/include/vlmo_hip.h b/include/vlmo_hip.h
--- a/include/vlmo_hip.h
+++ b/include/vlmo_hip.h
@@ -23,7 +23,8 @@
     VLMO_EPI_DUAL = 5,
     VLMO_EPI_ARGMAX = 6,
     VLMO_EPI_CE = 7,
-    VLMO_EPI_CE_BWD = 8
+    VLMO_EPI_CE_BWD = 8,
+    VLMO_EPI_BIAS_ROWDOT = 9
 };
 
 typedef struct VlmoEpilogue {
@@ -40,12 +41,15 @@
     uint32_t drop_thresh;
     float inv_keep;
     float beta;
-    uint64_t seed;
+    union {
+        uint64_t seed;
+        int64_t ldr;
+    };
     float* colpart;
 } VlmoEpilogue;
 
 const char* vlmo_last_error(void);
-#define VLMO_ABI_VERSION 16
+#define VLMO_ABI_VERSION 17
 int vlmo_abi_version(void);
 
 int vlmo_gemm_nt(int epi, int dtype, int tile, const void* A, int lda, const void* B, int ldb,
@@ -105,6 +109,11 @@
                   int lse_stride, const int32_t* seg, int num_seq, const int32_t* keymask,
                   void* dqkv, float* qv_colsum, int heads, int d, int max_len, float scale,
                   uint32_t drop_thresh, float inv_keep, uint64_t seed, int mask_seq0, hipStream_t stream);
+int vlmo_attn_bwd_rowdot(const void* qkv, const void* ctx, const void* dctx, const float* lse,
+                         int lse_stride, const int32_t* seg, int num_seq, const int32_t* keymask,
+                         void* dqkv, float* qv_colsum, int heads, int d, int max_len, float scale,
+                         uint32_t drop_thresh, float inv_keep, uint64_t seed, int mask_seq0,
+                         const float* rowdot, int rowdot_ld, hipStream_t stream);
 
 int vlmo_attn_probs(const void* qkv, const int32_t* seg, int num_seq, const int32_t* keymask, float* probs,
                     int heads, int d, int seq_len, int q0, int nq, int head_mean, float scale, hipStream_t stream);
```
